# Labbeti/conette-audio-captioning

Measured on AMD Instinct MI355X. Metric: clips_per_sec, higher is better.
Workload: dtype bf16; 1 GPU; B=64/GPU x 10 s @ 32 kHz clips, ConvNeXt encoder + beam-3 KV-cached decode (min 3 / max 20 tokens, V=5631), synthetic seeded checkpoint; batch_per_gpu=64, global_batch=64, beam_size=3, parallelism=dp1, world_size_observed=1, allreduce_of_ones=1, decode_group=2, decode_streams=2, encode_streams=1, input_batches_rotated=4

## Files before the change

conette-audio-captioning_amd/csrc/common.h:

```cpp
#pragma once
#include <hip/hip_runtime.h>
#include <stdint.h>
#include <stdio.h>
#include <string.h>
#include <mutex>
#include <set>
#include <utility>

typedef __bf16 bf16_t;
typedef __attribute__((ext_vector_type(8))) __bf16 bf16x8;
typedef __attribute__((ext_vector_type(4))) __bf16 bf16x4;
typedef __attribute__((ext_vector_type(4))) float f32x4;
typedef __attribute__((ext_vector_type(16))) float f32x16;

typedef _Float16 half_t;
template <typename H> using cn_h8 = H __attribute__((ext_vector_type(8)));
template <typename H> using cn_h4 = H __attribute__((ext_vector_type(4)));
typedef _Float16 cn_h2 __attribute__((ext_vector_type(2)));
template <typename T> struct CnIsH16 { static constexpr bool value = false; };
template <> struct CnIsH16<bf16_t> { static constexpr bool value = true; };
template <> struct CnIsH16<half_t> { static constexpr bool value = true; };
__device__ __forceinline__ f32x16 cn_mma32(cn_h8<bf16_t> a, cn_h8<bf16_t> b, f32x16 c) {
  return __builtin_amdgcn_mfma_f32_32x32x16_bf16(a, b, c, 0, 0, 0);
}
__device__ __forceinline__ f32x16 cn_mma32(cn_h8<half_t> a, cn_h8<half_t> b, f32x16 c) {
  return __builtin_amdgcn_mfma_f32_32x32x16_f16(a, b, c, 0, 0, 0);
}
__device__ __forceinline__ f32x4 cn_mma16(cn_h8<bf16_t> a, cn_h8<bf16_t> b, f32x4 c) {
  return __builtin_amdgcn_mfma_f32_16x16x32_bf16(a, b, c, 0, 0, 0);
}
__device__ __forceinline__ f32x4 cn_mma16(cn_h8<half_t> a, cn_h8<half_t> b, f32x4 c) {
  return __builtin_amdgcn_mfma_f32_16x16x32_f16(a, b, c, 0, 0, 0);
}
template <typename H> __device__ __forceinline__ cn_h8<H> cn_sat8(cn_h8<H> v) {
  if constexpr (__is_same(H, half_t)) {
    cn_h8<H> m;
#pragma unroll
    for (int i = 0; i < 8; ++i) m[i] = (H)65504.0f;
    return __builtin_elementwise_min(v, m);
  }
  return v;
}
template <typename H> __device__ __forceinline__ cn_h8<H> cn_pack8(float a, float b, float c, float d, float e, float f, float g, float h) {
  return cn_h8<H>{(H)a, (H)b, (H)c, (H)d, (H)e, (H)f, (H)g, (H)h};
}

__device__ __forceinline__ unsigned cn_lds_addr(const void* p) {
  return (unsigned)(size_t)(const __attribute__((address_space(3))) char*)p;
}
__device__ __forceinline__ void cn_dma16_v(const void* src_lane, unsigned lds) {
  asm volatile("s_mov_b32 m0, %1\n\tglobal_load_lds_dwordx4 %0, off" ::"v"(src_lane), "s"(lds) : "memory", "m0");
}
__device__ __forceinline__ void cn_dma16_s(const void* src_base, unsigned voff, unsigned lds) {
  asm volatile("s_mov_b32 m0, %2\n\tglobal_load_lds_dwordx4 %0, %1" ::"v"(voff), "s"(src_base), "s"(lds) : "memory", "m0");
}
__device__ __forceinline__ void cn_vm_wait(int n) {
#define CN_VM_CASE(N) case N: asm volatile("s_waitcnt vmcnt(" #N ")" ::: "memory"); break;
  switch (n) {
    CN_VM_CASE(0) CN_VM_CASE(1) CN_VM_CASE(2) CN_VM_CASE(3) CN_VM_CASE(4) CN_VM_CASE(5) CN_VM_CASE(6) CN_VM_CASE(7)
    CN_VM_CASE(8) CN_VM_CASE(9) CN_VM_CASE(10) CN_VM_CASE(11) CN_VM_CASE(12) CN_VM_CASE(13) CN_VM_CASE(14) CN_VM_CASE(15)
    CN_VM_CASE(16) CN_VM_CASE(17) CN_VM_CASE(18) CN_VM_CASE(19) CN_VM_CASE(20) CN_VM_CASE(21) CN_VM_CASE(22) CN_VM_CASE(23)
    CN_VM_CASE(24) CN_VM_CASE(25) CN_VM_CASE(26) CN_VM_CASE(27) CN_VM_CASE(28) CN_VM_CASE(29) CN_VM_CASE(30) CN_VM_CASE(31)
    CN_VM_CASE(32) CN_VM_CASE(33) CN_VM_CASE(34) CN_VM_CASE(35) CN_VM_CASE(36) CN_VM_CASE(37) CN_VM_CASE(38) CN_VM_CASE(39)
    CN_VM_CASE(40) CN_VM_CASE(41) CN_VM_CASE(42) CN_VM_CASE(43) CN_VM_CASE(44) CN_VM_CASE(45) CN_VM_CASE(46) CN_VM_CASE(47)
    CN_VM_CASE(48) CN_VM_CASE(49) CN_VM_CASE(50) CN_VM_CASE(51) CN_VM_CASE(52) CN_VM_CASE(53) CN_VM_CASE(54) CN_VM_CASE(55)
    CN_VM_CASE(56) CN_VM_CASE(57) CN_VM_CASE(58) CN_VM_CASE(59) CN_VM_CASE(60) CN_VM_CASE(61) CN_VM_CASE(62)
    default: break;
  }
#undef CN_VM_CASE
}

typedef __attribute__((ext_vector_type(2))) float f32x2;
typedef __attribute__((ext_vector_type(8))) _Float16 f16x8;
typedef __attribute__((ext_vector_type(4))) unsigned u32x4;

struct sp16_t {
  _Float16 hi, lo;
};
__device__ __forceinline__ unsigned cn_sp16_bits(float x) {
  x = __builtin_amdgcn_fmed3f(x, -65504.0f, 65504.0f);
  const _Float16 hi = (_Float16)x;
  const _Float16 lo = (_Float16)(x - (float)hi);
  return (unsigned)__builtin_bit_cast(unsigned short, hi) | ((unsigned)__builtin_bit_cast(unsigned short, lo) << 16);
}
__device__ __forceinline__ float cn_sp16_value(unsigned w) {
  return (float)__builtin_bit_cast(_Float16, (unsigned short)(w & 0xffffu)) + (float)__builtin_bit_cast(_Float16, (unsigned short)(w >> 16));
}

#define CN_OK 0
#define CN_ERR_ARG 1
#define CN_ERR_HIP 2
#define CN_ERR_WEIGHT 3
#define CN_ERR_WORKSPACE 4

void cn_set_error(const char* fmt, ...);

#define CN_HIP(expr)                                                                      \
  do {                                                                                    \
    hipError_t _e = (expr);                                                               \
    if (_e != hipSuccess) {                                                               \
      cn_set_error("%s:%d %s -> %s", __FILE__, __LINE__, #expr, hipGetErrorString(_e));   \
      return CN_ERR_HIP;                                                                  \
    }                                                                                     \
  } while (0)

#define CN_LAUNCH_CHECK()                                                                 \
  do {                                                                                    \
    hipError_t _e = hipGetLastError();                                                    \
    if (_e != hipSuccess) {                                                               \
      cn_set_error("%s:%d launch -> %s", __FILE__, __LINE__, hipGetErrorString(_e));      \
      return CN_ERR_HIP;                                                                  \
    }                                                                                     \
  } while (0)

#define CN_TRY(expr)                 \
  do {                               \
    int _s = (expr);                 \
    if (_s != CN_OK) return _s;      \
  } while (0)

static inline int cn_configure_lds(const void* fn, int bytes) {
  static std::mutex mu;
  static std::set<std::pair<int, const void*>> done;
  int dev = 0;
  CN_HIP(hipGetDevice(&dev));
  std::lock_guard<std::mutex> lock(mu);
  if (done.count(std::make_pair(dev, fn))) return CN_OK;
  CN_HIP(hipFuncSetAttribute(fn, hipFuncAttributeMaxDynamicSharedMemorySize, bytes));
  done.insert(std::make_pair(dev, fn));
  return CN_OK;
}

static inline size_t cn_align(size_t x, size_t a = 256) { return (x + a - 1) / a * a; }
static inline int cn_cdiv(int a, int b) { return (a + b - 1) / b; }

template <typename T> __device__ __forceinline__ T cn_from_f32(float x);
template <> __device__ __forceinline__ float cn_from_f32<float>(float x) { return x; }
template <> __device__ __forceinline__ bf16_t cn_from_f32<bf16_t>(float x) { return (bf16_t)x; }
template <> __device__ __forceinline__ half_t cn_from_f32<half_t>(float x) { return (half_t)__builtin_amdgcn_fmed3f(x, -65504.0f, 65504.0f); }
template <> __device__ __forceinline__ sp16_t cn_from_f32<sp16_t>(float x) { return __builtin_bit_cast(sp16_t, cn_sp16_bits(x)); }
__device__ __forceinline__ float cn_to_f32(float x) { return x; }
__device__ __forceinline__ float cn_to_f32(bf16_t x) { return (float)x; }
__device__ __forceinline__ float cn_to_f32(half_t x) { return (float)x; }
__device__ __forceinline__ float cn_to_f32(sp16_t x) { return (float)x.hi + (float)x.lo; }

__device__ __forceinline__ float cn_ld1(const float* p) { return *p; }
__device__ __forceinline__ float cn_ld1(const half_t* p) { return (float)*p; }
__device__ __forceinline__ f32x4 cn_ld4(const float* p) { return *(const f32x4*)p; }
__device__ __forceinline__ f32x4 cn_ld4(const half_t* p) {
  const cn_h4<half_t> h = *(const cn_h4<half_t>*)p;
  return f32x4{(float)h[0], (float)h[1], (float)h[2], (float)h[3]};
}

__device__ __forceinline__ float cn_gelu(float x) { return 0.5f * x * (1.0f + erff(x * 0.70710678118654752440f)); }

__device__ __forceinline__ float cn_gelu_fast(float x) {
  const float z = fabsf(x) * 0.70710678118654752440f;
  const float t = __builtin_amdgcn_rcpf(fmaf(0.3275911f, z, 1.0f));
  float p = fmaf(1.061405429f, t, -1.453152027f);
  p = fmaf(p, t, 1.421413741f);
  p = fmaf(p, t, -0.284496736f);
  p = fmaf(p, t, 0.254829592f);
  const float e = 1.0f - p * t * __expf(-z * z);
  return 0.5f * x + 0.5f * fabsf(x) * e;
}

__device__ __forceinline__ f32x2 cn_gelu_fast2(f32x2 x) {
  const f32x2 ax = __builtin_elementwise_abs(x);
  const f32x2 d = ax * (0.70710678118654752440f * 0.3275911f) + 1.0f;
  const f32x2 t = f32x2{__builtin_amdgcn_rcpf(d[0]), __builtin_amdgcn_rcpf(d[1])};
  f32x2 p = t * 1.061405429f + (-1.453152027f);
  p = p * t + 1.421413741f;
  p = p * t + (-0.284496736f);
  p = p * t + 0.254829592f;
  const f32x2 u = x * 0.84932180028801904272f;
  const f32x2 zz = -(u * u);
  const f32x2 e = f32x2{__builtin_amdgcn_exp2f(zz[0]), __builtin_amdgcn_exp2f(zz[1])};
  const f32x2 er = 1.0f - (p * t) * e;
  const f32x2 h = x * 0.5f;
  return __builtin_elementwise_abs(h) * er + h;
}
__device__ __forceinline__ f32x2 cn_gelu_as2(f32x2 x) {
  const f32x2 ax = __builtin_elementwise_abs(x);
  const f32x2 d = ax * (0.70710678118654752440f * 0.3275911f) + 1.0f;
  const f32x2 t = f32x2{__builtin_amdgcn_rcpf(d[0]), __builtin_amdgcn_rcpf(d[1])};
  f32x2 p = t * 1.061405429f + (-1.453152027f);
  p = p * t + 1.421413741f;
  p = p * t + (-0.284496736f);
  p = p * t + 0.254829592f;
  const f32x2 u = x * 0.84932180028801904272f;
  const f32x2 zz = -(u * u);
  const f32x2 e = f32x2{__builtin_amdgcn_exp2f(zz[0]), __builtin_amdgcn_exp2f(zz[1])};
  const f32x2 q = (p * t) * e;
  const f32x2 pos = f32x2{fmaxf(x[0], 0.f), fmaxf(x[1], 0.f)};
  return pos - (ax * 0.5f) * q;
}
__device__ __forceinline__ float cn_gelu_as(float x) { return cn_gelu_as2(f32x2{x, x})[0]; }
__device__ __forceinline__ f32x4 cn_gelu_as4(f32x4 x) {
  const f32x2 a = cn_gelu_as2(f32x2{x[0], x[1]}), b = cn_gelu_as2(f32x2{x[2], x[3]});
  return f32x4{a[0], a[1], b[0], b[1]};
}
__device__ __forceinline__ f32x4 cn_gelu_fast4(f32x4 x) {
  const f32x2 a = cn_gelu_fast2(f32x2{x[0], x[1]}), b = cn_gelu_fast2(f32x2{x[2], x[3]});
  return f32x4{a[0], a[1], b[0], b[1]};
}

template <int DEG> __device__ __forceinline__ float cn_gelu_e1_half(float h) {
  const float a = __builtin_fabsf(h);
  float p;
  if constexpr (DEG == 3) {
    p = fmaf(a, 8.0f * -0.02487156353890896f, 4.0f * -0.49887558817863464f);
    p = fmaf(p, a, 2.0f * -1.1291841268539429f);
    p = fmaf(p, a, 1.0f - 1.0035500526428223f);
  } else {
    static_assert(DEG == 5, "degree 3 or 5");
    p = fmaf(a, 32.0f * -0.0004728270578198135f, 16.0f * 0.007081141695380211f);
    p = fmaf(p, a, 8.0f * -0.05181875079870224f);
    p = fmaf(p, a, 4.0f * -0.4600019156932831f);
    p = fmaf(p, a, 2.0f * -1.1507835388183594f);
    p = fmaf(p, a, 1.0f - 1.0000382661819458f);
  }
  float g = fmaf(-a, __builtin_amdgcn_exp2f(p), h + a);
  asm("" : "+v"(g));
  return g;
}
// ... 74 lines not shown
```

conette-audio-captioning_amd/csrc/ctx.h:

```cpp
#pragma once
#include "../../include/conette_hip.h"
#include "common.h"

#define CN_N_MELS 224
#define CN_N_FFT 1024
#define CN_HOP 320
#define CN_N_BINS 513
#define CN_N_TAGS 527
#define CN_FEAT 768
#define CN_MAX_LAYERS 12

static const int CN_DEPTHS[4] = {3, 3, 9, 3};
static const int CN_DIMS[4] = {96, 192, 384, 768};

struct CnBlockW {
  const float* dw_w;
  const unsigned* dw_wp;
  const float* dw_b;
  const float* ln_w;
  const float* ln_b;
  const void* w1;
  const float* b1;
  const void* w2;
  const float* b2;
  const float* scale;
  const void* mlp_stream;
  const void* mlp_sp;
};

struct CnDownW {
  const float* ln_w;
  const float* ln_b;
  const void* w;
  const float* bias;
  const void* fused;
};

struct CnLayerW {
  const void* sa_in_w;
  const float* sa_in_b;
  const void* sa_out_w;
  const float* sa_out_b;
  const void* ca_q_w;
  const float* ca_q_b;
  const void* ca_out_w;
  const float* ca_out_b;
  const void* ff1_w;
  const float* ff1_b;
  const void* ff2_w;
  const float* ff2_b;
  const float *n1w, *n1b, *n2w, *n2b, *n3w, *n3b;
  const void* blk_w;
  const void* ffn_w;
  const float* blk_p;
};

struct CnRuntime;

struct conette_ctx {
  conette_config cfg;
  CnRuntime* rt;
  void* dec_graphs;
  unsigned long long serial;
  uint32_t prof_mask;
  int dec_unfused;
  int esize;
  int sp16;
  int f16;
  int no_encoder;
  const float* window;
  const float2* tw512;
  const float2* tw1024;
  const int* band;
  int mel_rows;
  const float* melC;
  const float* bn_scale;
  const float* bn_shift;
  const float* stem_w;
  const float* stem_b;
  const float* stem_ln_w;
  const float* stem_ln_b;
  CnBlockW blocks[18];
  CnDownW down[3];
  const float* norm_w;
  const float* norm_b;
  const void* head_w;
  const float* head_b;
  const void* proj_w;
  const float* proj_b;
  const void* kv_w;
  const float* kv_b;
  CnLayerW layers[CN_MAX_LAYERS];
  const float* emb;
  const float* pe;
  int pe_len;
  const void* cls_w;
  const float* cls_b;
  int n_cu;
  int enc_reserved_cus;
  int forcing_stepwise;
  int score_vsplit;
  char* arena;
  size_t arena_bytes;
  size_t arena_used;
};

void cn_prof_begin(conette_ctx* ctx, int cls, hipStream_t s);
void cn_prof_end(conette_ctx* ctx, int cls, hipStream_t s);
struct CnProfScope {
  conette_ctx* ctx;
  int cls;
  hipStream_t s;
  CnProfScope(conette_ctx* c, int k, hipStream_t st) : ctx(c), cls(k), s(st) {
    if (ctx->prof_mask & (1u << cls)) cn_prof_begin(ctx, cls, s);
  }
  ~CnProfScope() {
    if (ctx->prof_mask & (1u << cls)) cn_prof_end(ctx, cls, s);
  }
};

int cn_frontend(conette_ctx* ctx, const float* wave, int B, int L, float* out, hipStream_t s);

#define CN_BY_PRECISION(ctx, ...)                                                          \
  do {                                                                                     \
    switch ((ctx)->cfg.precision) {                                                        \
      case CONETTE_PREC_BF16: { typedef bf16_t OT; return __VA_ARGS__; }                   \
      case CONETTE_PREC_F16: { typedef half_t OT; return __VA_ARGS__; }                    \
      case CONETTE_PREC_F16X2: { typedef sp16_t OT; return __VA_ARGS__; }                  \
      default: { typedef float OT; return __VA_ARGS__; }                                   \
    }                                                                                      \
  } while (0)
#define CN_H16_CALL(ctx, ...)                          \
  do {                                                 \
    if ((ctx)->f16) { typedef half_t HT; __VA_ARGS__; } \
    else { typedef bf16_t HT; __VA_ARGS__; }            \
  } while (0)
```

conette-audio-captioning_amd/csrc/decoder.hip:

```cpp
#include "ctx.h"
#include <stdlib.h>

#include <type_traits>

#include "gemm2.h"
#include "dec_ffn.h"
#include "dec_score.h"
#include "dec_rows.h"
#include "dec_search.h"
#include "dec_sample.h"
#include "dec_group.h"
#include "dec_constrain.h"
#include "dec_require.h"
#include "dec_align.h"
#include "dec_ensemble.h"

#define FF2_SPLITS 8
static int ff2_splits_default() { return 4; }


struct DecWs {
  void *fe_t, *mem, *kvc, *xt, *attn_t, *ffh, *kc, *vc;
  float *x, *x2, *qkv, *q, *tmp, *logits, *slabs;
  int *n_active, *slot, *prefix, *anc, *cur_tok, *out_len, *eos_idx;
// ... 368 lines not shown
    if (step == 0 && a.step0_logits)
      CN_HIP(hipMemcpyAsync(a.step0_logits, w.logits, (size_t)R * w.ldv * 4, hipMemcpyDeviceToDevice, s));
    if (forcing) {
      hipLaunchKernelGGL(cn_force_store_kernel, dim3(cn_cdiv(V, 1024), R), dim3(256), 0, s, w.logits, w.ldv, V, maxp, step,
                         a.force_logits);
      CN_LAUNCH_CHECK();
      continue;
    }
    if (a.greedy_logits) {
      hipLaunchKernelGGL(cn_greedy_logits_kernel, dim3(cn_cdiv(V, 1024), B), dim3(256), 0, s, ss, step, cfg.pad_id, a.greedy_logits);
      CN_LAUNCH_CHECK();
    }
    CnProfScope ps_search(ctx, CONETTE_PROF_SEARCH, s);
    if (sampling) {
      SmArgs sa;
      sa.logits = w.logits, sa.forbid = a.forbid, sa.uniforms = a.uniforms, sa.prefix = w.prefix, sa.cur_tok = w.cur_tok;
      sa.sum_lp = w.sum_lp, sa.fin = w.slot, sa.live = w.live, sa.preds = a.mult_preds, sa.sum_out = a.mult_lprobs;
      sa.lens = a.sample_lens, sa.sizes = a.out_sizes, sa.tok_lp = a.sample_tok_lp, sa.step_logits = a.sample_step_logits;
      sa.ldv = w.ldv, sa.V = V, sa.R = R, sa.maxp = maxp, sa.min_pred = min_pred, sa.eos_id = cfg.eos_id, sa.top_k = a.top_k;
      sa.temperature = a.temperature, sa.top_p = a.top_p;
      const int vpt = cn_cdiv(V, SM_T);
#define SM_LAUNCH(VPT_) hipLaunchKernelGGL((cn_sample_step_kernel<VPT_>), dim3(R), dim3(SM_T), 0, s, sa, step)
      if (vpt <= 2) SM_LAUNCH(2);
      else if (vpt <= 4) SM_LAUNCH(4);
      else if (vpt <= 6) SM_LAUNCH(6);
      else if (vpt <= SM_VPT) SM_LAUNCH(8);
      else SM_LAUNCH(0);
#undef SM_LAUNCH
      CN_LAUNCH_CHECK();
      continue;
    }
    if (grouped) {
      cn_group_step_launch(ss, gs, B, step, s);
      CN_LAUNCH_CHECK();
      continue;
    }
    if (a.constrained) {
      if (a.req_width > 0) cn_require_step_launch(ss, cs, rq, B, step, s);
      else cn_constrain_step_launch(ss, cs, B, step, s);
      CN_LAUNCH_CHECK();
      continue;
    }
    if (V <= S3_T * S3_VPT && beam <= 8) {
#define S3_LAUNCH(NR_, VPT_) hipLaunchKernelGGL((cn_search_step3_kernel<NR_, VPT_>), dim3(B), dim3(S3_T), 0, s, ss, step)
      const int vpt = cn_cdiv(V, S3_T);
      if (beam <= 4) {
        if (vpt <= 2) S3_LAUNCH(4, 2);
        else if (vpt <= 4) S3_LAUNCH(4, 4);
        else if (vpt <= 6) S3_LAUNCH(4, 6);
        else S3_LAUNCH(4, 8);
      } else {
        if (vpt <= 4) S3_LAUNCH(8, 4);
        else S3_LAUNCH(8, 8);
      }
#undef S3_LAUNCH
    } else {
      hipLaunchKernelGGL(cn_search_step_kernel, dim3(B), dim3(256), 0, s, ss, step);
    }
    CN_LAUNCH_CHECK();
  }
  if (forcing || sampling) return CN_OK;
  hipLaunchKernelGGL(cn_finalize_kernel, dim3(cn_cdiv(B, 64)), dim3(64), 0, s, B, beam, maxp, cfg.eos_id, a.mult_preds,
                     a.mult_lprobs, w.out_len, a.best_preds, a.best_lprobs, w.eos_idx, a.out_sizes, a.margins);
  CN_LAUNCH_CHECK();
  hipLaunchKernelGGL(cn_finalize2_kernel, dim3(1), dim3(256), 0, s, B, w.eos_idx, a.out_sizes);
  CN_LAUNCH_CHECK();
  return CN_OK;
}

struct DecGraph {
  DecArgs key;
  hipGraphExec_t exec;
  hipGraph_t graph;
  hipEvent_t last;
  int seen;
  int nodes;
};
static void dec_graph_release(DecGraph& g) {
  if (!g.exec) return;
  if (g.last) {
    if (hipEventSynchronize(g.last) != hipSuccess) (void)hipGetLastError();
    (void)hipEventDestroy(g.last);
  }
  (void)hipGraphExecDestroy(g.exec);
  (void)hipGraphDestroy(g.graph);
  g.exec = nullptr, g.graph = nullptr, g.last = nullptr;
}
#define CN_MAX_DEC_GRAPHS 64
struct DecGraphCache {
  std::mutex mu;
  DecGraph g[CN_MAX_DEC_GRAPHS] = {};
  int n = 0;
  int enabled = 1;
  int last_nodes = 0;
};
static std::mutex g_dec_cache_create_mu;
static DecGraphCache* graph_cache(conette_ctx* ctx, bool create) {
  std::lock_guard<std::mutex> lock(g_dec_cache_create_mu);
  if (ctx->dec_graphs == nullptr && create) ctx->dec_graphs = new DecGraphCache();
  return (DecGraphCache*)ctx->dec_graphs;
}
void cn_decode_graphs_free(conette_ctx* ctx) {
  DecGraphCache* c = graph_cache(ctx, false);
  if (!c) return;
  {
    std::lock_guard<std::mutex> lock(c->mu);
    for (int i = 0; i < c->n; ++i) dec_graph_release(c->g[i]);
    c->n = 0;
  }
  std::lock_guard<std::mutex> lock(g_dec_cache_create_mu);
  delete c;
  ctx->dec_graphs = nullptr;
}
extern "C" int conette_set_option(conette_ctx* ctx, int32_t option, int32_t value) {
  if (!ctx) return CN_ERR_ARG;
  if (option == CONETTE_OPT_DECODE_GRAPH) {
    DecGraphCache* c = graph_cache(ctx, true);
    if (c) {
      std::lock_guard<std::mutex> lock(c->mu);
      c->enabled = value ? 1 : 0;
    }
    return CN_OK;
  }
  if (option == CONETTE_OPT_DECODE_FUSION) {
    ctx->dec_unfused = value ? 0 : 1;
    DecGraphCache* c = graph_cache(ctx, false);
    if (c) {
      std::lock_guard<std::mutex> lock(c->mu);
      for (int i = 0; i < c->n; ++i) dec_graph_release(c->g[i]);
      c->n = 0;
    }
    return CN_OK;
  }
  if (option == CONETTE_OPT_FORCING_STEPWISE) {
    ctx->forcing_stepwise = value ? 1 : 0;
    return CN_OK;
  }
  if (option == CONETTE_OPT_SCORE_VSPLIT) {
    if (value < 0) {
      cn_set_error("set_option: score vocabulary split %d < 0", value);
      return CN_ERR_ARG;
    }
    ctx->score_vsplit = value;
    return CN_OK;
  }
  if (option == CONETTE_OPT_ENCODE_RESERVED_CUS) {
    if (value < 0 || value > ctx->n_cu / 2) {
      cn_set_error("set_option: reserved CUs %d outside 0 .. %d", value, ctx->n_cu / 2);
      return CN_ERR_ARG;
    }
    ctx->enc_reserved_cus = value;
    return CN_OK;
  }
  cn_set_error("set_option: unknown option %d", option);
  return CN_ERR_ARG;
}

template <typename... A>
static int dec_check_model(const conette_ctx* ctx, const char* who, int len, int min_pred, const char* len_fmt, A... len_args) {
  if (len < 1 || len > CN_MAX_PRED || len > ctx->pe_len || min_pred < 0) {
    cn_set_error(len_fmt, len_args...);
    return CN_ERR_ARG;
  }
  if (ctx->cfg.d_model != 256 || ctx->cfg.nhead != 8) {
    cn_set_error("%s: kernels are specialised for d_model=256, nhead=8", who);
    return CN_ERR_ARG;
  }
  return CN_OK;
}
static int dec_check_workspace(const char* who, size_t workspace_bytes, size_t need) {
  if (workspace_bytes < need) {
    cn_set_error("%s: workspace %zu < %zu", who, workspace_bytes, need);
    return CN_ERR_WORKSPACE;
  }
  return CN_OK;
}

static int dec_check_search(const char* who, const int32_t* frame_lens, int batch, int t_audio, int beam, int min_pred, int max_pred,
                            const int32_t* best_preds, const float* best_lprobs, const int32_t* mult_preds, const float* mult_lprobs,
                            const int32_t* out_sizes) {
  if (!frame_lens || !best_preds || !best_lprobs || !mult_preds || !mult_lprobs || !out_sizes || batch <= 0 || t_audio <= 0) {
    cn_set_error("%s: bad argument", who);
    return CN_ERR_ARG;
  }
  if (beam < 1 || beam > CN_MAX_BEAM || max_pred < 1 || max_pred > CN_MAX_PRED || min_pred < 0) {
    cn_set_error("%s: beam=%d (1..%d) max_pred=%d (1..%d) min_pred=%d unsupported", who, beam, CN_MAX_BEAM, max_pred, CN_MAX_PRED,
                 min_pred);
    return CN_ERR_ARG;
  }
  return CN_OK;
}
static int dec_check_member(const char* who, const conette_ctx* ctx, int min_pred, int max_pred, size_t workspace_bytes, size_t need) {
  CN_TRY(dec_check_model(ctx, who, max_pred, min_pred, "%s: max_pred exceeds positional table", who));
  return dec_check_workspace(who, workspace_bytes, need);
}

template <typename Run>
static int dec_graph_run(conette_ctx* ctx, const DecArgs& key, hipStream_t s, Run run) {
  DecGraphCache* cache = graph_cache(ctx, true);
  const uint32_t dec_classes = (1u << CONETTE_PROF_DEC_PREPARE) | (1u << CONETTE_PROF_DEC_GEMM) |
                               (1u << CONETTE_PROF_DEC_ATTN) | (1u << CONETTE_PROF_DEC_MISC) |
                               (1u << CONETTE_PROF_SEARCH);
  if (!cache || (ctx->prof_mask & dec_classes) != 0) return run();

  auto find = [&]() -> DecGraph* {
    for (int i = 0; i < cache->n; ++i)
      if (cache->g[i].key == key) {
        const DecGraph hit = cache->g[i];
        memmove(&cache->g[i], &cache->g[i + 1], sizeof(DecGraph) * (cache->n - 1 - i));
        cache->g[cache->n - 1] = hit;
        return &cache->g[cache->n - 1];
      }
    return nullptr;
  };
  enum { EAGER, CAPTURE } todo = EAGER;
  DecGraph evicted;
  memset(&evicted, 0, sizeof(evicted));
  {
    std::lock_guard<std::mutex> lock(cache->mu);
    if (!cache->enabled) {
      todo = EAGER;
    } else if (DecGraph* e = find()) {
      if (e->exec) {
        CN_HIP(hipGraphLaunch(e->exec, s));
        CN_HIP(hipEventRecord(e->last, s));
        cache->last_nodes = e->nodes;
        return CN_OK;
      }
      if (e->seen == 1) {
        e->seen = 2;
        todo = CAPTURE;
      }
    } else {
      if (cache->n == CN_MAX_DEC_GRAPHS) {
        evicted = cache->g[0];
        memmove(&cache->g[0], &cache->g[1], sizeof(DecGraph) * (CN_MAX_DEC_GRAPHS - 1));
        cache->n--;
      }
      DecGraph* fresh = &cache->g[cache->n++];
      memset(fresh, 0, sizeof(*fresh));
      memcpy(&fresh->key, &key, sizeof(key));
      fresh->seen = 1;
    }
  }
  dec_graph_release(evicted);
  if (todo == EAGER) return run();

  hipGraph_t graph = nullptr;
  hipGraphExec_t exec = nullptr;
  hipEvent_t last = nullptr;
  auto capture = [&]() -> bool {
    if (hipStreamBeginCapture(s, hipStreamCaptureModeRelaxed) != hipSuccess) return false;
    const int rc = run();
    if (hipStreamEndCapture(s, &graph) != hipSuccess || rc != CN_OK || graph == nullptr) return false;
    if (hipGraphInstantiate(&exec, graph, nullptr, nullptr, 0) != hipSuccess || exec == nullptr) return false;
    return hipEventCreateWithFlags(&last, hipEventDisableTiming) == hipSuccess;
  };
  if (!capture()) {
    (void)hipGetLastError();
    if (exec) (void)hipGraphExecDestroy(exec);
    if (graph) (void)hipGraphDestroy(graph);
    {
      std::lock_guard<std::mutex> lock(cache->mu);
      cache->enabled = 0;
    }
    return run();
  }
  size_t n_nodes = 0;
  if (hipGraphGetNodes(graph, nullptr, &n_nodes) != hipSuccess) (void)hipGetLastError();
  {
    std::lock_guard<std::mutex> lock(cache->mu);
    DecGraph* e = find();
    if (e && !e->exec) {
      e->exec = exec, e->graph = graph, e->last = last, e->nodes = (int)n_nodes;
      cache->last_nodes = e->nodes;
      CN_HIP(hipGraphLaunch(exec, s));
      CN_HIP(hipEventRecord(last, s));
      return CN_OK;
    }
  }
  CN_HIP(hipGraphLaunch(exec, s));
  CN_HIP(hipEventRecord(last, s));
  DecGraph tmp;
  memset(&tmp, 0, sizeof(tmp));
  tmp.exec = exec, tmp.graph = graph, tmp.last = last;
  dec_graph_release(tmp);
  return CN_OK;
}

extern "C" int conette_decode(conette_ctx* ctx, const float* frame_embs, const int32_t* frame_lens,
                              const int32_t* bos_ids, const uint8_t* forbid_mask, int32_t batch, int32_t t_audio,
                              int32_t beam, int32_t min_pred, int32_t max_pred, int32_t* best_preds,
                              float* best_lprobs, int32_t* mult_preds, float* mult_lprobs, int32_t* out_sizes,
                              float* step0_logits, int32_t* trace_sel, float* trace_val, float* margins,
                              void* workspace, size_t workspace_bytes, void* stream) {
  if (!ctx || !frame_embs || !bos_ids || !workspace) {
    cn_set_error("decode: bad argument");
    return CN_ERR_ARG;
  }
  CN_TRY(dec_check_search("decode", frame_lens, batch, t_audio, beam, min_pred, max_pred, best_preds, best_lprobs, mult_preds, mult_lprobs,
                          out_sizes));
  CN_TRY(dec_check_member("decode", ctx, min_pred, max_pred, workspace_bytes, conette_decode_workspace_bytes(ctx, batch, t_audio, beam, max_pred)));
  DecArgs a;
  memset(&a, 0, sizeof(a));
  a.frame_embs = frame_embs, a.frame_lens = frame_lens, a.bos_ids = bos_ids, a.forbid = forbid_mask;
  a.best_preds = best_preds, a.best_lprobs = best_lprobs, a.mult_preds = mult_preds, a.mult_lprobs = mult_lprobs;
// ... 573 lines not shown
```

conette-audio-captioning_amd/csrc/encoder.hip:

```cpp
#include <stddef.h>

#include "ctx.h"
#include <type_traits>

__device__ int g_cn_nonfinite;
__device__ __forceinline__ void cn_watch_stat(float v) {
  if (!(__builtin_fabsf(v) <= 3.0e38f)) atomicAdd(&g_cn_nonfinite, 1);
}

#include "gemm2.h"
#include "mlp_rc2.h"
#include "mlp_rs16.h"
#include "mlp_sp.h"
#include "down_fused.h"

template <typename XT>
__global__ __launch_bounds__(256) void cn_stem_mfma_kernel(const float* __restrict__ in, int F, int H0, long n_pos,
                                                           const float* __restrict__ w , const float* __restrict__ bias,
                                                           const float* __restrict__ ln_w, const float* __restrict__ ln_b,
                                                           XT* __restrict__ out) {
  __shared__ __attribute__((aligned(16))) float s_p[3 * 96];
  for (int i = threadIdx.x; i < 3 * 96; i += 256) s_p[i] = i < 96 ? bias[i] : i < 192 ? ln_w[i - 96] : ln_b[i - 192];
  const int lane = threadIdx.x & 63, j = lane & 31, h = lane >> 5;
  float a[3][8];
#pragma unroll
  for (int t = 0; t < 3; ++t)
#pragma unroll
    for (int s = 0; s < 8; ++s) a[t][s] = w[(4 * (s >> 1) + 2 * h + (s & 1)) * 96 + 32 * t + cn_rc2_chan(j)];
  __syncthreads();
  const long n_tiles = (n_pos + 31) >> 5;
  const long n_waves = (long)gridDim.x * 4;
  for (long tile = (long)blockIdx.x * 4 + (threadIdx.x >> 6); tile < n_tiles; tile += n_waves) {
    const long pos = tile * 32 + j;
    const long p = pos < n_pos ? pos : n_pos - 1;
    const int wq = (int)(p % 56);
    const long tt = p / 56;
    const int hh = (int)(tt % H0);
    const int b = (int)(tt / H0);
    f32x2 xv[4];
#pragma unroll
    for (int i = 0; i < 4; ++i) {
      const int r = 4 * hh - 4 + i;
      xv[i] = f32x2{0.f, 0.f};
      if (r >= 0 && r < F) xv[i] = *(const f32x2*)(in + ((size_t)b * F + r) * CN_N_MELS + 4 * wq + 2 * h);
    }
    f32x16 acc[3];
#pragma unroll
    for (int t = 0; t < 3; ++t)
#pragma unroll
      for (int u = 0; u < 2; ++u) {
        const f32x4 b0 = *(const f32x4*)(s_p + 32 * t + 16 * u + 8 * h), b1 = *(const f32x4*)(s_p + 32 * t + 16 * u + 8 * h + 4);
#pragma unroll
        for (int e = 0; e < 4; ++e) acc[t][8 * u + e] = b0[e], acc[t][8 * u + 4 + e] = b1[e];
      }
#pragma unroll
    for (int s = 0; s < 8; ++s)
#pragma unroll
      for (int t = 0; t < 3; ++t) acc[t] = __builtin_amdgcn_mfma_f32_32x32x2f32(a[t][s], xv[s >> 1][s & 1], acc[t], 0, 0, 0);
    float sum = 0.f;
#pragma unroll
    for (int t = 0; t < 3; ++t)
#pragma unroll
      for (int r = 0; r < 16; ++r) sum += acc[t][r];
    sum += __shfl_xor(sum, 32);
    const float mean = sum * (1.0f / 96.0f);
    float v2 = 0.f;
#pragma unroll
    for (int t = 0; t < 3; ++t)
#pragma unroll
      for (int r = 0; r < 16; ++r) {
        acc[t][r] -= mean;
        v2 = fmaf(acc[t][r], acc[t][r], v2);
      }
    v2 += __shfl_xor(v2, 32);
    const float rstd = 1.0f / sqrtf(v2 * (1.0f / 96.0f) + 1e-6f);
    if (pos < n_pos) {
      XT* o = out + (size_t)pos * 96 + 8 * h;
#pragma unroll
      for (int t = 0; t < 3; ++t)
#pragma unroll
        for (int u = 0; u < 2; ++u) {
          const int ch = 32 * t + 16 * u + 8 * h;
          float v[8];
#pragma unroll
          for (int q = 0; q < 2; ++q) {
            const f32x4 lw = *(const f32x4*)(s_p + 96 + ch + 4 * q), lb = *(const f32x4*)(s_p + 192 + ch + 4 * q);
#pragma unroll
            for (int e = 0; e < 4; ++e) v[4 * q + e] = acc[t][8 * u + 4 * q + e] * rstd * lw[e] + lb[e];
          }
          if constexpr (sizeof(XT) == 2) {
            *(cn_h8<XT>*)(o + 32 * t + 16 * u) = cn_h8<XT>{cn_from_f32<XT>(v[0]), cn_from_f32<XT>(v[1]), cn_from_f32<XT>(v[2]), cn_from_f32<XT>(v[3]),
                                                          cn_from_f32<XT>(v[4]), cn_from_f32<XT>(v[5]), cn_from_f32<XT>(v[6]), cn_from_f32<XT>(v[7])};
          } else {
            *(f32x4*)(o + 32 * t + 16 * u) = f32x4{v[0], v[1], v[2], v[3]};
            *(f32x4*)(o + 32 * t + 16 * u + 4) = f32x4{v[4], v[5], v[6], v[7]};
          }
        }
    }
  }
}

__device__ unsigned long long g_dw_prof[8];
#define DW_STAMP(i)                                                   \
  if (dbg) {                                                          \
    const unsigned long long t_ = clock64();                          \
    if ((threadIdx.x & 63) == 0) atomicAdd(&g_dw_prof[i], t_ - t_prev); \
    t_prev = t_;                                                      \
  }

template <int C, int S, int TH> struct DwTile {
  static constexpr int NCHUNK = C / 4;
  static constexpr int PITCH4 = NCHUNK | 1;
  static constexpr int PITCH = PITCH4 * 4;
};

template <typename T, typename XT, int C, int S, int TH>
__global__ __launch_bounds__((C > 384 ? 384 : C) * S) void cn_dwconv_ln_kernel(const XT* __restrict__ x, int H, int W, int tiles_h,
                                                            int tiles_w, const float* __restrict__ dw_w ,
                                                            const unsigned* __restrict__ dw_wp ,
                                                            const float* __restrict__ dw_b,
                                                            const float* __restrict__ ln_w,
                                                            const float* __restrict__ ln_b, T* __restrict__ y,
                                                            int dbg) {
  extern __shared__ __attribute__((aligned(16))) char smem_raw[];
  float* s_v = (float*)smem_raw;
  unsigned long long t_prev = dbg ? clock64() : 0;
  constexpr int NP = TH * 4;
  constexpr int CT = C > 384 ? 384 : C;
  constexpr int PITCH = DwTile<C, S, TH>::PITCH;
  const int tid = threadIdx.x;
  const int c0 = tid % CT, sidx = tid / CT;
  int bid = cn_xcd_remap(blockIdx.x, gridDim.x);
  const int tw = bid % tiles_w;
  bid /= tiles_w;
  const int th = bid % tiles_h;
  const int b = bid / tiles_h;
  const int h0 = th * TH, w0 = tw * (4 * S) + sidx * 4;

  int wcl[10];
  bool wok[10];
#pragma unroll
  for (int q = 0; q < 10; ++q) {
    const int ww = w0 - 3 + q;
    wok[q] = (ww >= 0) && (ww < W);
    wcl[q] = min(max(ww, 0), W - 1) * C;
  }
#pragma unroll 1
  for (int c = c0; c < C; c += CT) {
  float acc[TH][4];
  const float bias = dw_b[c];
#pragma unroll
  for (int a = 0; a < TH; ++a)
#pragma unroll
    for (int e = 0; e < 4; ++e) acc[a][e] = bias;
  const XT* xb = x + (size_t)b * H * W * C + c;
  const bool interior = (h0 >= 3) && (h0 + TH + 3 <= H) && (w0 >= 3) && (w0 + 4 + 3 <= W);
  if constexpr (sizeof(XT) == 2) {
    static_assert(TH % 2 == 0, "row pairs");
    cn_h2 ke[3][7], ko[3][7];
#pragma unroll
    for (int a = 0; a < 3; ++a)
#pragma unroll
      for (int j = 0; j < 7; ++j) {
        ke[a][j] = __builtin_bit_cast(cn_h2, dw_wp[(a * 7 + j) * C + c]);
        ko[a][j] = __builtin_bit_cast(cn_h2, dw_wp[(21 + a * 7 + j) * C + c]);
      }
    DW_STAMP(0)
    auto fma_pair = [&](int r, const cn_h2 (&p)[10]) {
#pragma unroll
      for (int oh = 0; oh < TH; ++oh) {
        const int i = r - oh;
        if (i < -1 || i > 6) continue;
#pragma unroll
        for (int q = 0; q < 10; ++q)
#pragma unroll
          for (int ow = 0; ow < 4; ++ow) {
            const int j = q - ow;
            if (j < 0 || j > 6) continue;
            if (i == -1) acc[oh][ow] = fmaf((float)p[q][1], (float)ke[0][j][0], acc[oh][ow]);
            else if (i == 6) acc[oh][ow] = fmaf((float)p[q][0], (float)ko[2][j][1], acc[oh][ow]);
            else if ((i & 1) == 0) acc[oh][ow] = __builtin_amdgcn_fdot2(p[q], ke[i >> 1][j], acc[oh][ow], false);
            else acc[oh][ow] = __builtin_amdgcn_fdot2(p[q], ko[i >> 1][j], acc[oh][ow], false);
          }
      }
    };
    constexpr int NPR = (TH + 6) / 2;
    if (interior) {
      const XT* base = xb + ((size_t)(h0 - 3) * W + (w0 - 3)) * C;
      auto load_pair = [&](int r, cn_h2 (&p)[10]) {
        const XT* x0 = base + (size_t)r * W * C;
        const XT* x1 = x0 + (size_t)W * C;
#pragma unroll
        for (int q = 0; q < 10; ++q) p[q] = cn_h2{x0[q * C], x1[q * C]};
      };
      cn_h2 pa[10], pb[10];
      load_pair(0, pa);
#pragma unroll
      for (int u = 0; u < NPR; u += 2) {
        if (u + 1 < NPR) load_pair(2 * (u + 1), pb);
        fma_pair(2 * u, pa);
        if (u + 2 < NPR) load_pair(2 * (u + 2), pa);
        if (u + 1 < NPR) fma_pair(2 * (u + 1), pb);
      }
    } else {
#pragma unroll
      for (int u = 0; u < NPR; ++u) {
        const int hh0 = h0 - 3 + 2 * u, hh1 = hh0 + 1;
        const bool ok0 = (hh0 >= 0) && (hh0 < H), ok1 = (hh1 >= 0) && (hh1 < H);
        const XT* x0 = xb + (size_t)min(max(hh0, 0), H - 1) * W * C;
        const XT* x1 = xb + (size_t)min(max(hh1, 0), H - 1) * W * C;
        XT v0[10], v1[10];
#pragma unroll
        for (int q = 0; q < 10; ++q) v0[q] = x0[wcl[q]], v1[q] = x1[wcl[q]];
        cn_h2 p[10];
#pragma unroll
        for (int q = 0; q < 10; ++q) p[q] = cn_h2{(ok0 && wok[q]) ? v0[q] : (XT)0.f, (ok1 && wok[q]) ? v1[q] : (XT)0.f};
        fma_pair(2 * u, p);
      }
    }
  } else {
  float k[49];
#pragma unroll
  for (int i = 0; i < 49; ++i) k[i] = dw_w[i * C + c];
  DW_STAMP(0)
  auto fma_row = [&](int r, const XT (&v)[10]) {
#pragma unroll
    for (int oh = 0; oh < TH; ++oh) {
      const int i = r - oh;
      if (i < 0 || i > 6) continue;
#pragma unroll
      for (int q = 0; q < 10; ++q)
#pragma unroll
        for (int ow = 0; ow < 4; ++ow) {
          const int j = q - ow;
          if (j < 0 || j > 6) continue;
          acc[oh][ow] = fmaf((float)v[q], k[i * 7 + j], acc[oh][ow]);
        }
    }
  };
  if (interior) {
    const XT* base = xb + ((size_t)(h0 - 3) * W + (w0 - 3)) * C;
    XT va[10], vb[10];
#pragma unroll
    for (int q = 0; q < 10; ++q) va[q] = base[q * C];
#pragma unroll
    for (int r = 0; r < TH + 6; r += 2) {
      if (r + 1 < TH + 6) {
        const XT* xr = base + (size_t)(r + 1) * W * C;
#pragma unroll
        for (int q = 0; q < 10; ++q) vb[q] = xr[q * C];
      }
// ... 444 lines not shown
  }
  if (__syncthreads_or(bad ? 1 : 0) && threadIdx.x == 0) atomicAdd(&g_cn_nonfinite, 1);
}

template <typename T>
__global__ __launch_bounds__(256) void cn_clip_pool_ln_kernel(const float* __restrict__ fe, int Tn,
                                                              const float* __restrict__ ln_w,
                                                              const float* __restrict__ ln_b, T* __restrict__ out) {
  __shared__ float s_red[8];
  const int b = blockIdx.x, tid = threadIdx.x;
  float v[3];
  float s = 0.f;
#pragma unroll
  for (int i = 0; i < 3; ++i) {
    const int c = tid + 256 * i;
    float mx = -INFINITY, sm = 0.f;
    const float* col = fe + (size_t)b * Tn * CN_FEAT + c;
    int t = 0;
    for (; t + 8 <= Tn; t += 8) {
      float a[8];
#pragma unroll
      for (int u = 0; u < 8; ++u) a[u] = col[(size_t)(t + u) * CN_FEAT];
#pragma unroll
      for (int u = 0; u < 8; ++u) {
        mx = fmaxf(mx, a[u]);
        sm += a[u];
      }
    }
    for (; t < Tn; ++t) {
      const float a = col[(size_t)t * CN_FEAT];
      mx = fmaxf(mx, a);
      sm += a;
    }
    v[i] = mx + sm / (float)Tn;
    s += v[i];
  }
  s = cn_wave_sum(s);
  if ((tid & 63) == 0) s_red[tid >> 6] = s;
  __syncthreads();
  const float mean = (s_red[0] + s_red[1] + s_red[2] + s_red[3]) * (1.0f / CN_FEAT);
  float s2 = 0.f;
#pragma unroll
  for (int i = 0; i < 3; ++i) {
    const float d = v[i] - mean;
    s2 = fmaf(d, d, s2);
  }
  s2 = cn_wave_sum(s2);
  if ((tid & 63) == 0) s_red[4 + (tid >> 6)] = s2;
  __syncthreads();
  const float rstd = 1.0f / sqrtf((s_red[4] + s_red[5] + s_red[6] + s_red[7]) * (1.0f / CN_FEAT) + 1e-6f);
#pragma unroll
  for (int i = 0; i < 3; ++i) {
    const int c = tid + 256 * i;
    out[(size_t)b * CN_FEAT + c] = cn_from_f32<T>((v[i] - mean) * rstd * ln_w[c] + ln_b[c]);
  }
}

#ifndef CN_SP_NW96
#define CN_SP_NW96 12
#define CN_SP_NST96 4
#endif

struct EncGeom {
  int F, H[4], W[4];
};
static EncGeom enc_geom(int L) {
  EncGeom g;
  g.F = L / CN_HOP + 1;
  g.H[0] = (g.F + 8 - 4) / 4 + 1;
  g.W[0] = 56;
  for (int i = 1; i < 4; ++i) {
    g.H[i] = g.H[i - 1] / 2;
    g.W[i] = g.W[i - 1] / 2;
  }
  return g;
}

extern "C" int32_t conette_num_frames(int32_t n_samples) { return n_samples / CN_HOP + 1; }
extern "C" int32_t conette_num_audio_frames(int32_t n_samples) { return enc_geom(n_samples).H[3]; }

struct EncWs {
  float* logmel;
  void* x;
  void* y;
  void* h;
  void* fe_t;
  void* clip_t;
  size_t total;
};
static EncWs enc_ws(const conette_ctx* ctx, int B, int L, char* base) {
  const EncGeom g = enc_geom(L);
  const size_t es = ctx->esize;
  const size_t n0 = (size_t)B * g.H[0] * g.W[0] * 96;
  EncWs w;
  size_t off = 0;
  auto take = [&](size_t bytes) {
    char* p = base ? base + off : nullptr;
    off += cn_align(bytes);
    return p;
  };
  w.logmel = (float*)take((size_t)B * g.F * CN_N_MELS * 4);
  w.x = take((n0 + 32 * 96) * 4);
  w.y = take((n0 + 32 * 96) * es);
  w.h = take(n0 * 4 * es);
  w.fe_t = take((size_t)B * g.H[3] * CN_FEAT * es);
  w.clip_t = take((size_t)B * CN_FEAT * es);
  w.total = off;
  return w;
}

extern "C" size_t conette_encode_workspace_bytes(const conette_ctx* ctx, int32_t batch, int32_t n_samples) {
  return enc_ws(ctx, batch, n_samples, nullptr).total;
}

template <typename T, typename XT>
static int dwconv_dispatch(int C, const XT* x, int B, int H, int W, const CnBlockW& bw, T* y, hipStream_t s) {
  switch (C) {
    case 96: return launch_dwconv<T, XT, 96, CN_DW96_S, sizeof(XT) == 2 ? CN_DW96_TH : 8>(x, B, H, W, bw, y, s);
    case 192: return launch_dwconv<T, XT, 192, CN_DW192_S, sizeof(XT) == 2 ? CN_DW192_TH : 8>(x, B, H, W, bw, y, s);
    case 384:
      if (W == 14) return launch_dwconv_fw<T, XT, 384, 14, CN_FW_TH, CN_FW_SPLIT>(x, B, H, bw, y, s);
      return launch_dwconv<T, XT, 384, 1, 4>(x, B, H, W, bw, y, s);
    case 768:
      if (W == 7) return launch_dwconv_fw<T, XT, 768, 7, 4>(x, B, H, bw, y, s);
      return launch_dwconv<T, XT, 768, 1, 4>(x, B, H, W, bw, y, s);
  }
  cn_set_error("dwconv: unsupported C=%d", C);
  return CN_ERR_ARG;
}

static int tap_copy(float* dst, const float* src, size_t n, hipStream_t s) {
  if (dst) CN_HIP(hipMemcpyAsync(dst, src, n * sizeof(float), hipMemcpyDeviceToDevice, s));
  return CN_OK;
}
static __global__ void cn_tap_widen_kernel(const half_t* __restrict__ src, float* __restrict__ dst, size_t n) {
  for (size_t i = (size_t)blockIdx.x * blockDim.x + threadIdx.x; i < n; i += (size_t)gridDim.x * blockDim.x) dst[i] = (float)src[i];
}
static int tap_copy(float* dst, const half_t* src, size_t n, hipStream_t s) {
  if (dst) {
    hipLaunchKernelGGL(cn_tap_widen_kernel, dim3((unsigned)((n + 255) / 256 < 4096 ? (n + 255) / 256 : 4096)), dim3(256), 0, s, src, dst, n);
    CN_LAUNCH_CHECK();
  }
  return CN_OK;
}

template <typename T, typename XT>
static int encode_impl(conette_ctx* ctx, const float* wave, int B, int L, float* frame_embs, float* clip_probs,
                       const conette_encode_taps* taps, char* wsp, hipStream_t s) {
  const EncGeom g = enc_geom(L);
  EncWs ws = enc_ws(ctx, B, L, wsp);
  T* y = (T*)ws.y;
  T* hbuf = (T*)ws.h;
  XT* const wsx = (XT*)ws.x;
  {
    CnProfScope ps(ctx, CONETTE_PROF_FRONTEND, s);
    CN_TRY(cn_frontend(ctx, wave, B, L, ws.logmel, s));
  }
  if (taps) CN_TRY(tap_copy(taps->logmel, ws.logmel, (size_t)B * g.F * CN_N_MELS, s));
  {
    const long n_pos = (long)B * g.H[0] * g.W[0];
    CnProfScope ps(ctx, CONETTE_PROF_STEM, s);
    const long n_tiles = (n_pos + 31) / 32;
    const unsigned grid = (unsigned)std::min<long>((n_tiles + 3) / 4, 8L * ctx->n_cu);
    hipLaunchKernelGGL((cn_stem_mfma_kernel<XT>), dim3(grid), dim3(256), 0, s, ws.logmel, g.F, g.H[0], n_pos, ctx->stem_w, ctx->stem_b,
                       ctx->stem_ln_w, ctx->stem_ln_b, wsx);
    CN_LAUNCH_CHECK();
    if (taps) CN_TRY(tap_copy(taps->stem, wsx, (size_t)n_pos * 96, s));
  }
  XT* xc = wsx;
  int blk = 0;
  for (int st = 0; st < 4; ++st) {
    const int C = CN_DIMS[st], H = g.H[st], W = g.W[st];
    const long P = (long)B * H * W;
    if (st > 0) {
      const int Cp = CN_DIMS[st - 1], Hp = g.H[st - 1], Wp = g.W[st - 1];
      const long n_in = (long)B * Hp * Wp;
      const CnDownW& dw = ctx->down[st - 1];
      CnProfScope ps(ctx, CONETTE_PROF_DOWNSAMPLE, s);
      bool fused_down = false;
      if constexpr (CnIsH16<T>::value) if (Cp <= 192 && dw.fused != nullptr) {
        XT* xo = xc == wsx ? (XT*)ws.h : wsx;
        const int nb = ctx->n_cu - ctx->enc_reserved_cus;
        if (Cp == 96) CN_TRY((cn_launch_down_fused<96, 8, T, XT>(xc, B, Hp, Wp, dw.fused, xo, nb, s)));
        else CN_TRY((cn_launch_down_fused_ring<192, 4, 4, 3, T, XT>(xc, B, Hp, Wp, dw.fused, xo, nb, s)));
        xc = xo;
        if (taps) CN_TRY(tap_copy(taps->down[st], xc, (size_t)P * C, s));
        fused_down = true;
      }
      if (!fused_down) {
      const int ppb = Cp == 96 ? 32 : 16;
      const dim3 pg((unsigned)((n_in + ppb - 1) / ppb));
      if (Cp == 96)
        hipLaunchKernelGGL((cn_ln_patchify_kernel<T, XT, 96>), pg, dim3(256), 0, s, xc, Hp, Wp, n_in, dw.ln_w, dw.ln_b, y);
      else if (Cp == 192)
        hipLaunchKernelGGL((cn_ln_patchify_kernel<T, XT, 192>), pg, dim3(256), 0, s, xc, Hp, Wp, n_in, dw.ln_w, dw.ln_b, y);
      else
        hipLaunchKernelGGL((cn_ln_patchify_kernel<T, XT, 384>), pg, dim3(256), 0, s, xc, Hp, Wp, n_in, dw.ln_w, dw.ln_b, y);
      CN_LAUNCH_CHECK();
      EpiBiasAct<XT, ACT_NONE> epi{dw.bias, wsx, C, ACT_NONE};
      CN_TRY(cn_mm(y, 4 * Cp, (const T*)dw.w, 4 * Cp, (int)P, C, 4 * Cp, epi, s));
      xc = wsx;
      if (taps) CN_TRY(tap_copy(taps->down[st], xc, (size_t)P * C, s));
      }
    }
    for (int b = 0; b < CN_DEPTHS[st]; ++b, ++blk) {
      const CnBlockW& bw = ctx->blocks[blk];
      {
        CnProfScope ps(ctx, CONETTE_PROF_DWCONV_LN, s);
        CN_TRY((dwconv_dispatch<T, XT>(C, xc, B, H, W, bw, y, s)));
      }
      bool fused = false;
      if constexpr (std::is_same<T, sp16_t>::value) {
        if (bw.mlp_sp != nullptr && C <= 192) {
          CnProfScope ps(ctx, CONETTE_PROF_PW1_GEMM, s);
          const int nb = ctx->n_cu - ctx->enc_reserved_cus;
          if (C == 96) CN_TRY((cn_launch_mlp_sp_ring<96, CN_SP_NW96, CN_SP_NST96>(y, bw.mlp_sp, xc, (int)P, nb, s)));
          else CN_TRY((cn_launch_mlp_sp_ring<192, 8, 3>(y, bw.mlp_sp, xc, (int)P, nb, s)));
          fused = true;
        }
      }
      if constexpr (CnIsH16<T>::value) if (!fused) {
        if (bw.mlp_stream != nullptr && C <= 384) {
          CnProfScope ps(ctx, CONETTE_PROF_PW1_GEMM, s);
          const T* wsm = (const T*)bw.mlp_stream;
          if (C == 96) CN_TRY((cn_launch_mlp_rc2_resident<96, 12, 1>(y, wsm, xc, (int)P, ctx->n_cu - ctx->enc_reserved_cus, s)));
          else if (C == 192) CN_TRY((cn_launch_mlp_rc2_ring<192, 8, CN_RC2_NCK(192), CN_RC2_NCK(192) == 2 ? 3 : 5>(y, wsm, xc, (int)P, ctx->n_cu - ctx->enc_reserved_cus, s)));
          else CN_TRY((cn_launch_mlp_rs16<384, 4, 3, 8>(y, wsm, xc, (int)P, ctx->n_cu - ctx->enc_reserved_cus, s)));
          fused = true;
        }
      }
      if (!fused) {
        {
          CnProfScope ps(ctx, CONETTE_PROF_PW1_GEMM, s);
          constexpr int kAct = CnGeluAct<T>::value;
          EpiBiasAct<T, kAct> e1{bw.b1, hbuf, 4 * C, kAct};
          CN_TRY(cn_mm(y, C, (const T*)bw.w1, C, (int)P, 4 * C, C, e1, s));
        }
        {
          CnProfScope ps(ctx, CONETTE_PROF_PW2_GEMM, s);
          EpiResidT<XT> e2{bw.b2, bw.scale, xc, xc, C};
          CN_TRY(cn_mm(hbuf, 4 * C, (const T*)bw.w2, 4 * C, (int)P, C, 4 * C, e2, s));
        }
      }
      if (taps && b == 0) CN_TRY(tap_copy(taps->stage_block0[st], xc, (size_t)P * C, s));
      if (taps && taps->struct_bytes >= offsetof(conette_encode_taps, block) + (size_t)(blk + 1) * sizeof(float*))
        CN_TRY(tap_copy(taps->block[blk], xc, (size_t)P * C, s));
    }
    if (taps) CN_TRY(tap_copy(taps->stage[st], xc, (size_t)P * C, s));
  }
  const int Tn = g.H[3];
  CnProfScope ps_heads(ctx, CONETTE_PROF_HEADS, s);
  hipLaunchKernelGGL((cn_frame_mean_kernel<T, XT>), dim3((unsigned)(B * Tn)), dim3(256), 0, s, xc, g.W[3], CN_FEAT,
                     frame_embs, (T*)nullptr);
  CN_LAUNCH_CHECK();
  if (clip_probs) {
    hipLaunchKernelGGL((cn_clip_pool_ln_kernel<T>), dim3((unsigned)B), dim3(256), 0, s, frame_embs, Tn, ctx->norm_w,
                       ctx->norm_b, (T*)ws.clip_t);
    CN_LAUNCH_CHECK();
    EpiBiasAct<float> eh{ctx->head_b, clip_probs, CN_N_TAGS, ACT_SIGMOID};
    CN_TRY(cn_mm((const T*)ws.clip_t, CN_FEAT, (const T*)ctx->head_w, CN_FEAT, B, CN_N_TAGS, CN_FEAT, eh, s));
  }
  return CN_OK;
}

extern "C" int conette_encode_nonfinite(conette_ctx* ctx, void* stream, int32_t* count) {
  if (!ctx || !count) {
    cn_set_error("encode_nonfinite: bad argument");
    return CN_ERR_ARG;
  }
  hipStream_t s = (hipStream_t)stream;
  int32_t host = 0;
  CN_HIP(hipMemcpyFromSymbolAsync(&host, HIP_SYMBOL(g_cn_nonfinite), sizeof(host), 0, hipMemcpyDeviceToHost, s));
  CN_HIP(hipStreamSynchronize(s));
  if (host != 0) {
    const int32_t zero = 0;
    CN_HIP(hipMemcpyToSymbolAsync(HIP_SYMBOL(g_cn_nonfinite), &zero, sizeof(zero), 0, hipMemcpyHostToDevice, s));
    CN_HIP(hipStreamSynchronize(s));
  }
  *count = host;
  return CN_OK;
}

extern "C" int conette_frontend_logmel(conette_ctx* ctx, const float* wave, int32_t batch, int32_t n_samples,
                                       float* out, void* stream) {
  if (!ctx || !wave || !out || batch <= 0) {
    cn_set_error("frontend_logmel: bad argument");
    return CN_ERR_ARG;
  }
  if (ctx->no_encoder) {
    cn_set_error("frontend_logmel: decoder-only context (created without preprocessor.encoder.* tensors)");
    return CN_ERR_ARG;
  }
  return cn_frontend(ctx, wave, batch, n_samples, out, (hipStream_t)stream);
}

extern "C" int conette_encode(conette_ctx* ctx, const float* wave, int32_t batch, int32_t n_samples,
                              float* frame_embs, float* clip_probs, const conette_encode_taps* taps, void* workspace,
                              size_t workspace_bytes, void* stream) {
  if (conette_num_audio_frames(n_samples) < 1) {
    cn_set_error("encode: n_samples=%d is too short: the encoder's three 2x downsamplings need >= 7680 samples "
                 "(0.24 s at 32 kHz) to leave one audio frame", n_samples);
    return CN_ERR_ARG;
  }
  if (!ctx || !wave || !frame_embs || !workspace || batch <= 0) {
    cn_set_error("encode: bad argument");
    return CN_ERR_ARG;
  }
  if (ctx->no_encoder) {
    cn_set_error("encode: decoder-only context (created without preprocessor.encoder.* tensors: a BaselinePLM-layout checkpoint "
                 "takes precomputed frame embeddings)");
    return CN_ERR_ARG;
  }
  if (taps && taps->struct_bytes < offsetof(conette_encode_taps, block)) {
    cn_set_error("encode: conette_encode_taps.struct_bytes = %zu is smaller than the version-1 members (%zu): set it to "
                 "sizeof(conette_encode_taps)", taps->struct_bytes, offsetof(conette_encode_taps, block));
    return CN_ERR_ARG;
  }
  const size_t need = conette_encode_workspace_bytes(ctx, batch, n_samples);
  if (workspace_bytes < need) {
    cn_set_error("encode: workspace %zu < %zu", workspace_bytes, need);
    return CN_ERR_WORKSPACE;
// ... 13 lines not shown
```

conette-audio-captioning_amd/csrc/frontend.hip:

```cpp
#include "ctx.h"

__device__ __forceinline__ float2 cmul(float2 a, float2 b) { return float2{a.x * b.x - a.y * b.y, a.x * b.y + a.y * b.x}; }
__device__ __forceinline__ float2 cadd(float2 a, float2 b) { return float2{a.x + b.x, a.y + b.y}; }
__device__ __forceinline__ float2 csub(float2 a, float2 b) { return float2{a.x - b.x, a.y - b.y}; }
__device__ __forceinline__ float2 cmul_mi(float2 a) { return float2{a.y, -a.x}; }

__device__ __forceinline__ void dft8(float2 (&v)[8]) {
  const float h = 0.70710678118654752440f;
  float2 a[8];
#pragma unroll
  for (int i = 0; i < 4; ++i) {
    a[i] = cadd(v[i], v[i + 4]);
    a[i + 4] = csub(v[i], v[i + 4]);
  }
  a[5] = float2{h * (a[5].x + a[5].y), h * (a[5].y - a[5].x)};
  a[6] = cmul_mi(a[6]);
  a[7] = float2{h * (a[7].y - a[7].x), -h * (a[7].x + a[7].y)};
  float2 b0 = cadd(a[0], a[2]), b2 = csub(a[0], a[2]), b1 = cadd(a[1], a[3]), b3 = cmul_mi(csub(a[1], a[3]));
  float2 b4 = cadd(a[4], a[6]), b6 = csub(a[4], a[6]), b5 = cadd(a[5], a[7]), b7 = cmul_mi(csub(a[5], a[7]));
  v[0] = cadd(b0, b1);
  v[4] = csub(b0, b1);
  v[2] = cadd(b2, b3);
  v[6] = csub(b2, b3);
  v[1] = cadd(b4, b5);
  v[5] = csub(b4, b5);
  v[3] = cadd(b6, b7);
  v[7] = csub(b6, b7);
}

__device__ __forceinline__ void cn_wave_sync() { __builtin_amdgcn_wave_barrier(); }

#define FE_PITCH 72

#ifndef FE_NW
#define FE_NW 16
#endif
#define FE_STATIC_BYTES ((512 + 513) * 8 + 1024 * 4 + FE_NW * 8 * FE_PITCH * 8 + FE_NW * 520 * 4)
#define FE_LDS_TOTAL (160 * 1024)
#define FE_FILL_BYTES ((FE_LDS_TOTAL - FE_STATIC_BYTES - 256) / 256 * 256)
#define FE_MEL_LDS_MAX FE_FILL_BYTES
static_assert(FE_STATIC_BYTES + FE_FILL_BYTES > FE_LDS_TOTAL - 768 && FE_STATIC_BYTES + FE_FILL_BYTES <= FE_LDS_TOTAL,
              "the log-mel block must own its compute unit's LDS");
template <bool MEL_LDS>
__global__ __launch_bounds__(FE_NW * 64) void cn_logmel_kernel(const float* __restrict__ wave, int L, int F, int total, int mel_rows,
                                                        const float* __restrict__ window,
                                                        const float2* __restrict__ tw512,
                                                        const float2* __restrict__ tw1024,
                                                        const float* __restrict__ melC, const int* __restrict__ band,
                                                        const float* __restrict__ bn_scale,
                                                        const float* __restrict__ bn_shift, float* __restrict__ out) {
  __shared__ float2 s_tw512[512];
  __shared__ float2 s_tw1024[513];
  __shared__ __attribute__((aligned(16))) float s_win[1024];
  __shared__ float2 s_x[FE_NW][8 * FE_PITCH];
  __shared__ float s_p[FE_NW][520];
  extern __shared__ __attribute__((aligned(16))) float s_mel[];
  const int tid = threadIdx.x, lane = tid & 63, wv = tid >> 6;
  if (MEL_LDS)
    for (int i = tid; i < mel_rows * CN_N_MELS; i += FE_NW * 64) s_mel[i] = melC[i];
  for (int i = tid; i < 512; i += FE_NW * 64) s_tw512[i] = tw512[i];
  for (int i = tid; i < 513; i += FE_NW * 64) s_tw1024[i] = tw1024[i];
  for (int i = tid; i < 1024; i += FE_NW * 64) s_win[i] = window[i];
  __syncthreads();
  float2* sx = s_x[wv];
  float* sp = s_p[wv];
  int m_lo[4], m_trip[4];
  float m_sc[4], m_sh[4];
#pragma unroll
  for (int g = 0; g < 4; ++g) {
    const int m = lane + 64 * g;
    const bool on = m < CN_N_MELS;
    m_sc[g] = on ? bn_scale[m] : 0.f;
    m_sh[g] = on ? bn_shift[m] : 0.f;
    m_lo[g] = on ? band[2 * m] : 0;
    int nb = on ? band[2 * m + 1] - m_lo[g] : 0;
#pragma unroll
    for (int d = 32; d > 0; d >>= 1) nb = max(nb, __shfl_xor(nb, d));
    m_trip[g] = min(nb, mel_rows);
  }
  const bool pair_loads = (L & 1) == 0 && (((size_t)wave) & 7) == 0;

  for (int base = blockIdx.x * FE_NW; base < total; base += gridDim.x * FE_NW) {
    const int fr = base + wv;
    const bool act = fr < total;
    float2 v[8];
    if (act) {
      const int b = fr / F, f = fr - b * F;
      const float* x = wave + (size_t)b * L;
      const int p0 = f * CN_HOP - CN_N_FFT / 2;
      if (pair_loads && p0 >= 0 && p0 + CN_N_FFT <= L) {
#pragma unroll
        for (int a = 0; a < 8; ++a) {
          const int n2 = 2 * (64 * a + lane);
          const float2 xv = *(const float2*)(x + p0 + n2);
          const float2 wv2 = *(const float2*)(s_win + n2);
          v[a] = float2{xv.x * wv2.x, xv.y * wv2.y};
        }
      } else {
#pragma unroll
        for (int a = 0; a < 8; ++a) {
          const int n2 = 2 * (64 * a + lane);
          int q0 = p0 + n2, q1 = q0 + 1;
          q0 = q0 < 0 ? -q0 : (q0 >= L ? 2 * L - 2 - q0 : q0);
          q1 = q1 < 0 ? -q1 : (q1 >= L ? 2 * L - 2 - q1 : q1);
          v[a] = float2{x[q0] * s_win[n2], x[q1] * s_win[n2 + 1]};
        }
      }
    } else {
#pragma unroll
      for (int a = 0; a < 8; ++a) v[a] = float2{0.f, 0.f};
    }
    dft8(v);
#pragma unroll
    for (int c = 1; c < 8; ++c) v[c] = cmul(v[c], s_tw512[lane * c]);
#pragma unroll
    for (int c = 0; c < 8; ++c) sx[c * FE_PITCH + lane] = v[c];
    cn_wave_sync();
    const int c = lane >> 3, lo3 = lane & 7;
#pragma unroll
    for (int a = 0; a < 8; ++a) v[a] = sx[c * FE_PITCH + 8 * a + lo3];
    dft8(v);
#pragma unroll
    for (int cp = 1; cp < 8; ++cp) v[cp] = cmul(v[cp], s_tw512[8 * lo3 * cp]);
    cn_wave_sync();
#pragma unroll
    for (int cp = 0; cp < 8; ++cp) sx[c * FE_PITCH + cp * 8 + lo3] = v[cp];
    cn_wave_sync();
#pragma unroll
    for (int bp = 0; bp < 8; ++bp) v[bp] = sx[c * FE_PITCH + lo3 * 8 + bp];
    dft8(v);
    cn_wave_sync();
#pragma unroll
    for (int dp = 0; dp < 8; ++dp) sx[c + 8 * lo3 + 64 * dp] = v[dp];
    cn_wave_sync();
#pragma unroll
    for (int j = 0; j < 8; ++j) {
      const int k = lane + 64 * j;
      const float2 A = sx[k];
      const float2 Bz = sx[(512 - k) & 511];
      const float2 E = float2{0.5f * (A.x + Bz.x), 0.5f * (A.y - Bz.y)};
      const float2 O = float2{0.5f * (A.y + Bz.y), -0.5f * (A.x - Bz.x)};
      const float2 X = cadd(E, cmul(s_tw1024[k], O));
      sp[k] = X.x * X.x + X.y * X.y;
    }
    if (lane == 0) {
      const float2 A = sx[0];
      const float xr = A.x - A.y;
      sp[512] = xr * xr;
    }
    cn_wave_sync();
    if (act) {
#pragma unroll
      for (int g = 0; g < 4; ++g) {
        const int m = lane + 64 * g;
        if (m < CN_N_MELS) {
          const int lo = m_lo[g], trip = m_trip[g];
          const float* mc = MEL_LDS ? s_mel : melC;
          float acc = 0.f;
          int i = 0;
          for (; i + 4 <= trip; i += 4) {
            float p[4], w[4];
#pragma unroll
            for (int u = 0; u < 4; ++u) {
              p[u] = sp[min(lo + i + u, CN_N_BINS - 1)];
              w[u] = mc[(i + u) * CN_N_MELS + m];
            }
#pragma unroll
            for (int u = 0; u < 4; ++u) acc = fmaf(p[u], w[u], acc);
          }
          for (; i < trip; ++i) acc = fmaf(sp[min(lo + i, CN_N_BINS - 1)], mc[i * CN_N_MELS + m], acc);
          const float db = 10.0f * log10f(acc < 1e-10f ? 1e-10f : acc);
          out[(size_t)fr * CN_N_MELS + m] = db * m_sc[g] + m_sh[g];
        }
      }
    }
    cn_wave_sync();
  }
}

int cn_frontend(conette_ctx* ctx, const float* wave, int B, int L, float* out, hipStream_t s) {
  if (L <= CN_N_FFT / 2) {
    cn_set_error("frontend: n_samples=%d must exceed %d (reflect padding)", L, CN_N_FFT / 2);
    return CN_ERR_ARG;
  }
  const int F = L / CN_HOP + 1;
  const long total = (long)B * F;
  int grid = (int)((total + FE_NW - 1) / FE_NW);
  if (grid > ctx->n_cu) grid = ctx->n_cu;
  const int mel_bytes = ctx->mel_rows * CN_N_MELS * 4;
  if (mel_bytes <= FE_MEL_LDS_MAX) {
    const int dyn = FE_FILL_BYTES;
    CN_TRY(cn_configure_lds((const void*)cn_logmel_kernel<true>, dyn));
    hipLaunchKernelGGL(cn_logmel_kernel<true>, dim3(grid), dim3(FE_NW * 64), dyn, s, wave, L, F, (int)total, ctx->mel_rows,
                       ctx->window, ctx->tw512, ctx->tw1024, ctx->melC, ctx->band, ctx->bn_scale, ctx->bn_shift, out);
  } else {
    CN_TRY(cn_configure_lds((const void*)cn_logmel_kernel<false>, FE_FILL_BYTES));
    hipLaunchKernelGGL(cn_logmel_kernel<false>, dim3(grid), dim3(FE_NW * 64), FE_FILL_BYTES, s, wave, L, F, (int)total,
                       ctx->mel_rows, ctx->window, ctx->tw512, ctx->tw1024, ctx->melC, ctx->band, ctx->bn_scale, ctx->bn_shift, out);
  }
  CN_LAUNCH_CHECK();
  return CN_OK;
}
```

conette-audio-captioning_amd/csrc/mlp_rc2.h:

```cpp
#pragma once
#include "common.h"

template <int C, int NCK> struct Rc2Geom {
  static constexpr int KS1 = C / 16, NT2 = C / 32, NCH = C / 8;
  static constexpr int F1 = KS1 + 1, F2 = 2 * NT2;
  static constexpr int NSTEP = NCH / NCK;
  static constexpr int FRAGS = NCK * (F1 + F2);
  static constexpr int STEP_BYTES = FRAGS * 1024;
  static constexpr size_t STREAM_BYTES = (size_t)NSTEP * STEP_BYTES;
  static constexpr size_t TOTAL_BYTES = STREAM_BYTES + NT2 * 1024;
};
__host__ __device__ constexpr int cn_rc2_chan(int m) { return (m & 19) | ((m & 4) << 1) | ((m & 8) >> 1); }

#define CN_MLP_XSCALE 0.5f
template <typename HT> __device__ __forceinline__ float cn_gelu_mlp(float x) {
  return cn_gelu_e1_half<__is_same(HT, half_t) ? 5 : 3>(x);
}

template <typename HT>
static __global__ void pk_mlp_rc2(const float* __restrict__ W1, const float* __restrict__ b1, const float* __restrict__ W2,
                           const float* __restrict__ b2, const float* __restrict__ scale, int C, int NCK,
                           HT* __restrict__ dst) {
  const int KS1 = C / 16, NT2 = C / 32, NCH = C / 8, F1 = KS1 + 1, F2 = 2 * NT2, FRAGS = NCK * (F1 + F2), NSTEP = NCH / NCK;
  const int u = blockIdx.x * blockDim.x + threadIdx.x;
  if (u >= (NSTEP * FRAGS + NT2) * 64) return;
  const int l = u & 63, q = (u >> 6) % FRAGS, st = (u >> 6) / FRAGS;
  const int r = l & 31, h = l >> 5;
  float v[8];
  if (st >= NSTEP) {
    const int c = 32 * q + cn_rc2_chan(r);
    const float b = scale[c] * b2[c];
    const float hi = (float)(HT)b;
#pragma unroll
    for (int i = 0; i < 8; ++i) v[i] = 0.f;
    if (h == 0) {
      v[0] = hi;
      v[1] = b - hi;
    }
  } else if (q < NCK * F1) {
    const int j = st * NCK + q / F1, s = q % F1;
    if (s < KS1) {
#pragma unroll
      for (int i = 0; i < 8; ++i) v[i] = CN_MLP_XSCALE * W1[(size_t)(32 * j + r) * C + 16 * s + 8 * h + i];
    } else {
      const float b = CN_MLP_XSCALE * b1[32 * j + r];
      const float hi = (float)(HT)b;
#pragma unroll
      for (int i = 0; i < 8; ++i) v[i] = 0.f;
      if (h == 0) {
        v[0] = hi;
        v[1] = b - hi;
      }
    }
  } else {
    const int q2 = q - NCK * F1;
    const int j = st * NCK + q2 / F2, s = (q2 % F2) / NT2, t = (q2 % F2) % NT2;
    const int c = 32 * t + cn_rc2_chan(r);
    const float sc = scale[c];
#pragma unroll
    for (int i = 0; i < 8; ++i) v[i] = sc * W2[(size_t)c * (4 * C) + 32 * j + 16 * s + 8 * (i >> 2) + 4 * h + (i & 3)];
  }
#pragma unroll
  for (int i = 0; i < 8; ++i) dst[(size_t)u * 8 + i] = (HT)v[i];
}

#define CN_RC2_NCK(C) ((C) == 192 ? 2 : 1)


template <int C, int NCK, typename HT = bf16_t, typename XT = float> struct Rc2Wave {
  typedef Rc2Geom<C, NCK> G;
  typedef cn_h8<HT> hx8;
  static constexpr int KS1 = G::KS1, NT2 = G::NT2, F1 = G::F1, F2 = G::F2;

  static __device__ __forceinline__ hx8 frag(const char* wc, int f) { return *(const hx8*)(wc + f * 1024); }
  static __device__ __forceinline__ f32x16 mma(hx8 a, hx8 b, f32x16 c) { return cn_mma32(a, b, c); }
  static __device__ __forceinline__ hx8 gelu8(const f32x16& X, int o) {
    float g[8];
#pragma unroll
    for (int i = 0; i < 8; ++i) g[i] = cn_gelu_mlp<HT>(X[o + i]);
    return cn_sat8<HT>(cn_pack8<HT>(g[0], g[1], g[2], g[3], g[4], g[5], g[6], g[7]));
  }
  static __device__ __forceinline__ f32x16 zero16() {
    f32x16 z;
#pragma unroll
    for (int i = 0; i < 16; ++i) z[i] = 0.f;
    return z;
  }

  static constexpr int PRE = 4;
  static constexpr int NM = NCK * (F1 + F2), R = PRE + 1;
  struct State {
    hx8 F[R];
    f32x16 X[NCK];
    float g[NCK][16];
    hx8 H[NCK][2];
  };
  static constexpr int gelu_at(int i, int e) {
    if (NCK == 2) return i == 0 ? F1 + 1 + e * (F1 - 1) / 16 : 2 * F1 + e * F2 / 16;
    return e < 8 ? F1 - 1 : F1 + (e - 8) * NT2 / 8;
  }
  template <int Q, int I, int E>
  static __device__ __forceinline__ void gelu_slices(State& st) {
    if constexpr (gelu_at(I, E) == Q) {
      st.g[I][E] = cn_gelu_mlp<HT>(st.X[I][E]);
      if constexpr ((E & 7) == 7) {
        constexpr int o = E - 7;
        st.H[I][E >> 3] = cn_sat8<HT>(cn_pack8<HT>(st.g[I][o], st.g[I][o + 1], st.g[I][o + 2], st.g[I][o + 3],
                                                   st.g[I][o + 4], st.g[I][o + 5], st.g[I][o + 6], st.g[I][o + 7]));
      }
    }
    if constexpr (E + 1 < 16) gelu_slices<Q, I, E + 1>(st);
    else if constexpr (I + 1 < NCK) gelu_slices<Q, I + 1, 0>(st);
  }
  template <int Q>
  static __device__ __forceinline__ void mstep(const char* wc, const hx8 (&fy)[KS1], const hx8 ones, f32x16 (&O)[NT2],
                                               State& st) {
    if constexpr (Q + PRE < NM) st.F[(Q + PRE) % R] = frag(wc, Q + PRE);
    if constexpr (Q < NCK * F1) {
      constexpr int i = Q / F1, s = Q % F1;
      if constexpr (s == 0) st.X[i] = zero16();
      if constexpr (s < KS1) st.X[i] = mma(st.F[Q % R], fy[s], st.X[i]);
      else st.X[i] = mma(st.F[Q % R], ones, st.X[i]);
    } else {
      constexpr int q2 = Q - NCK * F1, i = q2 / F2, k = (q2 % F2) / NT2, t = q2 % NT2;
      O[t] = mma(st.F[Q % R], st.H[i][k], O[t]);
    }
    gelu_slices<Q, 0, 0>(st);
    __builtin_amdgcn_sched_barrier(0);
    if constexpr (Q + 1 < NM) mstep<Q + 1>(wc, fy, ones, O, st);
  }
  template <int Q>
  static __device__ __forceinline__ void prefetch(const char* wc, State& st) {
    st.F[Q % R] = frag(wc, Q);
    if constexpr (Q + 1 < PRE) prefetch<Q + 1>(wc, st);
  }
  static __device__ __forceinline__ void step(const char* wc, const hx8 (&fy)[KS1], const hx8 ones, f32x16 (&O)[NT2]) {
    State st;
    prefetch<0>(wc, st);
    __builtin_amdgcn_sched_barrier(0);
    mstep<0>(wc, fy, ones, O, st);
  }


  static __device__ __forceinline__ void load_y(const HT* __restrict__ Y, int m0, int lane, hx8 (&fy)[KS1]) {
    const HT* base = Y + (size_t)m0 * C;
    const int voff = (lane & 31) * C + 8 * (lane >> 5);
#pragma unroll
    for (int s = 0; s < KS1; ++s) fy[s] = *(const hx8*)(base + voff + 16 * s);
  }

  static __device__ __forceinline__ void init_o(const XT* __restrict__ X, const char* __restrict__ bbf, const hx8 ones, int m0,
                                                int lane, f32x16 (&O)[NT2]) {
    const XT* base = X + (size_t)m0 * C;
    const int voff = (lane & 31) * C + 8 * (lane >> 5);
    hx8 fb[NT2];
    if constexpr (sizeof(XT) == 2) {
      cn_h8<XT> v[NT2][2];
#pragma unroll
      for (int t = 0; t < NT2; ++t) {
        v[t][0] = *(const cn_h8<XT>*)(base + voff + 32 * t);
        v[t][1] = *(const cn_h8<XT>*)(base + voff + 32 * t + 16);
      }
#pragma unroll
      for (int t = 0; t < NT2; ++t) fb[t] = *(const hx8*)(bbf + t * 1024);
#pragma unroll
// ... 224 lines not shown
```

conette-audio-captioning_amd/engine.py:

```python
from __future__ import annotations

import ctypes as C
import os
from typing import Any, Dict, Optional, Tuple

import torch

_HERE = os.path.dirname(os.path.abspath(__file__))
LIB_PATH = os.path.join(_HERE, "libconette_hip.so")

PREC_F32 = 0
PREC_BF16 = 1
PREC_F16X2 = 2
PREC_F16 = 4
N_MELS = 224
FEAT = 768
N_TAGS = 527

EXPORTS = (
    "conette_last_error", "conette_abi_version", "conette_create", "conette_destroy", "conette_num_frames",
    "conette_num_audio_frames", "conette_encode_workspace_bytes", "conette_decode_workspace_bytes",
    "conette_frontend_logmel", "conette_encode", "conette_decode", "conette_resample", "conette_resample_len",
    "conette_set_option", "conette_profile_enable", "conette_profile_read", "conette_stream_create_masked",
    "conette_stream_destroy", "conette_forcing_workspace_bytes", "conette_forcing",
    "conette_greedy_workspace_bytes", "conette_greedy", "conette_decode_graph_nodes", "conette_encode_nonfinite",
    "conette_score_workspace_bytes", "conette_score", "conette_sample_workspace_bytes", "conette_sample",
    "conette_align_workspace_bytes", "conette_align", "conette_decode_groups_workspace_bytes", "conette_decode_groups",
    "conette_decode_constrained_workspace_bytes", "conette_decode_constrained",
    "conette_decode_required_workspace_bytes", "conette_decode_required",
    "conette_decode_ensemble_workspace_bytes", "conette_decode_ensemble",
)
CERT_TOL = {
    "mixed16": {"greedy": (0.032, 0.0, 0.0), "beam": (0.045, 0.0, 0.005), "wide": (0.08, 0.0, 0.005)},
    "f16": {"greedy": (0.063, 0.0, 0.0), "beam": (0.082, 0.0, 0.008), "wide": (0.13, 0.0, 0.008)},
    "bf16+f16dec": {"greedy": (0.20, 0.0, 0.0), "beam": (0.37, 0.0, 0.026), "wide": (0.65, 0.0, 0.05)},
    "bf16": {"greedy": (0.39, 0.0, 0.0), "beam": (0.58, 0.0, 0.05), "wide": (1.0, 0.0, 0.08)},
}


def cert_kind(beam: int) -> str:
    return "greedy" if int(beam) == 1 else ("beam" if int(beam) <= 5 else "wide")


CERT_DEFAULT_BASE = "mixed16"
OPT_DECODE_GRAPH = 1
OPT_DECODE_FUSION = 2
OPT_ENCODE_RESERVED_CUS = 3
OPT_FORCING_STEPWISE = 4
OPT_SCORE_VSPLIT = 5
MAX_DECODE_GRAPHS = 64
PROF_CLASSES = ("frontend", "stem", "dwconv_ln", "pw1_gemm", "pw2_gemm", "downsample", "heads", "dec_prepare",
                "dec_gemm", "dec_attn", "dec_misc", "search")


class ConetteConfigC(C.Structure):
    _fields_ = [(n, C.c_int32) for n in ("precision", "vocab_size", "d_model", "nhead", "n_layers", "d_ff", "pad_id",
                                         "bos_id", "eos_id")] + [("reserved", C.c_int32 * 7)]


class EncodeTapsC(C.Structure):
    _fields_ = [("struct_bytes", C.c_size_t), ("logmel", C.c_void_p), ("stem", C.c_void_p), ("stage_block0", C.c_void_p * 4),
                ("stage", C.c_void_p * 4), ("down", C.c_void_p * 4), ("block", C.c_void_p * 18)]


class ConetteMemberC(C.Structure):
    _fields_ = [("ctx", C.c_void_p), ("frame_embs", C.c_void_p), ("bos_ids", C.c_void_p), ("weight", C.c_float),
                ("workspace", C.c_void_p), ("workspace_bytes", C.c_size_t)]


_lib = None


def load_library() -> C.CDLL:
    global _lib
    if _lib is not None:
        return _lib
    if not os.path.exists(LIB_PATH):
        raise RuntimeError(
            f"{LIB_PATH} is missing: build it with `python -c 'import __graft_entry__ as g; g.build()'` "
            "(the MI355X path has no CPU fallback)")
    lib = C.CDLL(LIB_PATH)
    lib.conette_last_error.restype = C.c_char_p
    lib.conette_abi_version.restype = C.c_int
    lib.conette_create.restype = C.c_int
    lib.conette_create.argtypes = [C.POINTER(ConetteConfigC), C.c_int32, C.POINTER(C.c_char_p), C.POINTER(C.c_void_p),
                                   C.POINTER(C.c_int64), C.POINTER(C.c_void_p)]
    lib.conette_destroy.restype = None
    lib.conette_destroy.argtypes = [C.c_void_p]
    lib.conette_num_frames.restype = C.c_int32
    lib.conette_num_frames.argtypes = [C.c_int32]
    lib.conette_num_audio_frames.restype = C.c_int32
    lib.conette_num_audio_frames.argtypes = [C.c_int32]
    lib.conette_encode_workspace_bytes.restype = C.c_size_t
    lib.conette_encode_workspace_bytes.argtypes = [C.c_void_p, C.c_int32, C.c_int32]
    lib.conette_decode_workspace_bytes.restype = C.c_size_t
    lib.conette_decode_workspace_bytes.argtypes = [C.c_void_p, C.c_int32, C.c_int32, C.c_int32, C.c_int32]
    lib.conette_frontend_logmel.restype = C.c_int
    lib.conette_frontend_logmel.argtypes = [C.c_void_p, C.c_void_p, C.c_int32, C.c_int32, C.c_void_p, C.c_void_p]
    lib.conette_encode.restype = C.c_int
    lib.conette_encode.argtypes = [C.c_void_p, C.c_void_p, C.c_int32, C.c_int32, C.c_void_p, C.c_void_p,
                                   C.POINTER(EncodeTapsC), C.c_void_p, C.c_size_t, C.c_void_p]
    lib.conette_decode.restype = C.c_int
    lib.conette_decode.argtypes = [C.c_void_p, C.c_void_p, C.c_void_p, C.c_void_p, C.c_void_p, C.c_int32, C.c_int32,
                                   C.c_int32, C.c_int32, C.c_int32, C.c_void_p, C.c_void_p, C.c_void_p, C.c_void_p,
                                   C.c_void_p, C.c_void_p, C.c_void_p, C.c_void_p, C.c_void_p, C.c_void_p, C.c_size_t,
                                   C.c_void_p]
    lib.conette_encode_nonfinite.restype = C.c_int
    lib.conette_encode_nonfinite.argtypes = [C.c_void_p, C.c_void_p, C.POINTER(C.c_int32)]
    lib.conette_forcing_workspace_bytes.restype = C.c_size_t
    lib.conette_forcing_workspace_bytes.argtypes = [C.c_void_p, C.c_int32, C.c_int32, C.c_int32]
    lib.conette_forcing.restype = C.c_int
    lib.conette_forcing.argtypes = [C.c_void_p, C.c_void_p, C.c_void_p, C.c_void_p, C.c_int32, C.c_int32, C.c_int32,
                                    C.c_void_p, C.c_void_p, C.c_size_t, C.c_void_p]
    lib.conette_score_workspace_bytes.restype = C.c_size_t
    lib.conette_score_workspace_bytes.argtypes = [C.c_void_p, C.c_int32, C.c_int32, C.c_int32, C.c_int32]
    lib.conette_score.restype = C.c_int
    lib.conette_score.argtypes = [C.c_void_p, C.c_void_p, C.c_void_p, C.c_void_p, C.c_void_p, C.c_int32, C.c_int32, C.c_int32,
                                  C.c_int32, C.c_void_p, C.c_void_p, C.c_void_p, C.c_void_p, C.c_size_t, C.c_void_p]
    lib.conette_align_workspace_bytes.restype = C.c_size_t
    lib.conette_align_workspace_bytes.argtypes = [C.c_void_p, C.c_int32, C.c_int32, C.c_int32, C.c_int32, C.c_int32]
    lib.conette_align.restype = C.c_int
    lib.conette_align.argtypes = [C.c_void_p, C.c_void_p, C.c_void_p, C.c_void_p, C.c_void_p, C.c_int32, C.c_int32, C.c_int32,
                                  C.c_int32, C.c_uint32, C.c_void_p, C.c_void_p, C.c_void_p, C.c_void_p, C.c_void_p, C.c_void_p,
                                  C.c_size_t, C.c_void_p]
    lib.conette_sample_workspace_bytes.restype = C.c_size_t
    lib.conette_sample_workspace_bytes.argtypes = [C.c_void_p, C.c_int32, C.c_int32, C.c_int32, C.c_int32]
    lib.conette_sample.restype = C.c_int
    lib.conette_sample.argtypes = [C.c_void_p, C.c_void_p, C.c_void_p, C.c_void_p, C.c_void_p, C.c_void_p, C.c_int32, C.c_int32,
                                   C.c_int32, C.c_int32, C.c_int32, C.c_float, C.c_int32, C.c_float, C.c_void_p, C.c_void_p,
                                   C.c_void_p, C.c_void_p, C.c_void_p, C.c_void_p, C.c_void_p, C.c_size_t, C.c_void_p]
    lib.conette_decode_groups_workspace_bytes.restype = C.c_size_t
    lib.conette_decode_groups_workspace_bytes.argtypes = [C.c_void_p, C.c_int32, C.c_int32, C.c_int32, C.c_int32, C.c_int32]
    lib.conette_decode_groups.restype = C.c_int
    lib.conette_decode_groups.argtypes = [C.c_void_p, C.c_void_p, C.c_void_p, C.c_void_p, C.c_void_p, C.c_int32, C.c_int32, C.c_int32,
                                          C.c_int32, C.c_float, C.c_int32, C.c_int32, C.c_void_p, C.c_void_p, C.c_void_p, C.c_void_p,
                                          C.c_void_p, C.c_void_p, C.c_void_p, C.c_void_p, C.c_void_p, C.c_size_t, C.c_void_p]
    lib.conette_decode_constrained_workspace_bytes.restype = C.c_size_t
    lib.conette_decode_constrained_workspace_bytes.argtypes = [C.c_void_p, C.c_int32, C.c_int32, C.c_int32, C.c_int32]
    lib.conette_decode_constrained.restype = C.c_int
    lib.conette_decode_constrained.argtypes = [C.c_void_p, C.c_void_p, C.c_void_p, C.c_void_p, C.c_void_p, C.c_void_p, C.c_void_p,
                                               C.c_int32, C.c_void_p, C.c_int32, C.c_int32, C.c_int32, C.c_int32, C.c_int32,
                                               C.c_int32, C.c_void_p, C.c_void_p, C.c_void_p, C.c_void_p, C.c_void_p, C.c_void_p,
                                               C.c_void_p, C.c_void_p, C.c_void_p, C.c_size_t, C.c_void_p]
    lib.conette_decode_required_workspace_bytes.restype = C.c_size_t
    lib.conette_decode_required_workspace_bytes.argtypes = [C.c_void_p, C.c_int32, C.c_int32, C.c_int32, C.c_int32]
    lib.conette_decode_required.restype = C.c_int
    lib.conette_decode_required.argtypes = [C.c_void_p, C.c_void_p, C.c_void_p, C.c_void_p, C.c_void_p, C.c_void_p, C.c_void_p,
                                            C.c_int32, C.c_void_p, C.c_int32, C.c_void_p, C.c_void_p, C.c_int32, C.c_int32, C.c_int32,
                                            C.c_int32, C.c_int32, C.c_int32, C.c_void_p, C.c_void_p, C.c_void_p, C.c_void_p, C.c_void_p,
                                            C.c_void_p, C.c_void_p, C.c_void_p, C.c_void_p, C.c_size_t, C.c_void_p]
    lib.conette_decode_ensemble_workspace_bytes.restype = C.c_size_t
    lib.conette_decode_ensemble_workspace_bytes.argtypes = [C.c_void_p, C.c_int32, C.c_int32, C.c_int32, C.c_int32]
    lib.conette_decode_ensemble.restype = C.c_int
    lib.conette_decode_ensemble.argtypes = [C.POINTER(ConetteMemberC), C.c_int32, C.c_int32, C.c_void_p, C.c_void_p, C.c_int32, C.c_int32,
                                            C.c_int32, C.c_int32, C.c_int32, C.c_void_p, C.c_void_p, C.c_void_p, C.c_void_p, C.c_void_p,
                                            C.c_void_p, C.c_void_p, C.c_void_p, C.c_void_p, C.c_void_p]
    lib.conette_greedy_workspace_bytes.restype = C.c_size_t
    lib.conette_greedy_workspace_bytes.argtypes = [C.c_void_p, C.c_int32, C.c_int32, C.c_int32]
    lib.conette_greedy.restype = C.c_int
    lib.conette_greedy.argtypes = [C.c_void_p, C.c_void_p, C.c_void_p, C.c_void_p, C.c_void_p, C.c_int32, C.c_int32,
                                   C.c_int32, C.c_int32, C.c_void_p, C.c_void_p, C.c_void_p, C.c_void_p, C.c_size_t,
                                   C.c_void_p]
    lib.conette_set_option.restype = C.c_int
    lib.conette_set_option.argtypes = [C.c_void_p, C.c_int32, C.c_int32]
    lib.conette_decode_graph_nodes.restype = C.c_int32
    lib.conette_decode_graph_nodes.argtypes = [C.c_void_p]
    lib.conette_profile_enable.restype = C.c_int
    lib.conette_profile_enable.argtypes = [C.c_void_p, C.c_uint32]
    lib.conette_profile_read.restype = C.c_int
    lib.conette_profile_read.argtypes = [C.c_void_p, C.POINTER(C.c_float), C.POINTER(C.c_int32)]
    lib.conette_stream_create_masked.restype = C.c_int
    lib.conette_stream_create_masked.argtypes = [C.POINTER(C.c_uint32), C.c_int32, C.POINTER(C.c_void_p)]
    lib.conette_stream_destroy.restype = C.c_int
    lib.conette_stream_destroy.argtypes = [C.c_void_p]
    lib.conette_resample.restype = C.c_int
    lib.conette_resample.argtypes = [C.c_void_p, C.c_int32, C.c_int32, C.c_int32, C.c_int32, C.c_void_p, C.c_void_p]
    lib.conette_resample_len.restype = C.c_int32
    lib.conette_resample_len.argtypes = [C.c_int32, C.c_int32, C.c_int32]
    if lib.conette_abi_version() != 3:
        raise RuntimeError("libconette_hip.so ABI version mismatch")
    _lib = lib
    return lib


def _check(status: int, what: str) -> None:
    if status != 0:
        raise RuntimeError(f"{what} failed ({status}): {load_library().conette_last_error().decode()}")


def _stream() -> C.c_void_p:
    return C.c_void_p(torch.cuda.current_stream().cuda_stream)


def _ptr(t: Optional[torch.Tensor]) -> C.c_void_p:
    return C.c_void_p(0 if t is None else t.data_ptr())


def encoder_geometry(n_samples: int) -> Tuple[int, list, list]:
    f = n_samples // 320 + 1
    h = [(f + 8 - 4) // 4 + 1]
    w = [56]
    for _ in range(3):
# ... 5 lines not shown
def make_partitioned_streams(device: torch.device, decode_share: int = 8, n_cus: int = 256):
    lib = load_library()
    words = (n_cus + 31) // 32
    dec = [0] * words
    for i in range(0, n_cus, decode_share):
        dec[i // 32] |= 1 << (i % 32)
    enc = [(~w) & 0xFFFFFFFF for w in dec]
    out = []
    with torch.cuda.device(device):
        for mask in (enc, dec):
            h = C.c_void_p()
            _check(lib.conette_stream_create_masked((C.c_uint32 * words)(*mask), words, C.byref(h)),
                   "conette_stream_create_masked")
            out.append(torch.cuda.ExternalStream(h.value, device=device))
    return out[0], out[1]


def make_masked_stream(device: torch.device, n_share: int, n_cus: int = 256, offset: int = 0):
    lib = load_library()
    words = (n_cus + 31) // 32
    mask = [0] * words
    for j in range(n_share):
        i = (offset + j) % n_cus
        mask[i // 32] |= 1 << (i % 32)
    with torch.cuda.device(device):
        h = C.c_void_p()
        _check(lib.conette_stream_create_masked((C.c_uint32 * words)(*mask), words, C.byref(h)), "conette_stream_create_masked")
        return torch.cuda.ExternalStream(h.value, device=device)


def uncertified_mask(margins: torch.Tensor, best_lprobs: torch.Tensor, tol: Tuple[float, float, float], order: bool = True) -> torch.Tensor:
    a, b, c = tol
    max_pred = margins.shape[2] - 1
    need = a + b * torch.arange(1, max_pred + 1, device=margins.device, dtype=torch.float32)
    ok = (margins[:, 0, :max_pred] >= need).all(dim=1) & (margins[:, 0, max_pred] >= c) & torch.isfinite(best_lprobs)
    if order:
        ok = ok & (margins[:, 1, :max_pred] >= need).all(dim=1)
    return ~ok


def caption_sizes(best_preds: torch.Tensor, mult_preds: torch.Tensor, eos_id: int) -> torch.Tensor:
    max_pred = mult_preds.shape[-1]
    pos = torch.arange(max_pred, device=mult_preds.device)

    def first_eos(x):
        return torch.where(x == eos_id, pos, max_pred).amin(dim=-1)

    ps = torch.clamp(first_eos(mult_preds) + 1, max=max_pred).amax()
    e = first_eos(best_preds)
    ml = torch.minimum(torch.where(e < ps, e, ps).amax() + 1, ps)
    return torch.stack([ps, ml]).to(torch.int32)


class Engine:

    def __init__(self, state_dict: Dict[str, torch.Tensor], *, precision: str = "bf16", d_model: int = 256,
                 nhead: int = 8, n_layers: int = 6, d_ff: int = 2048, pad_id: int = 0, bos_id: int = 1,
                 eos_id: int = 2, device: Optional[torch.device] = None) -> None:
        if not torch.cuda.is_available():
            raise RuntimeError("conette_amd.Engine needs a ROCm GPU (no CPU fallback)")
        self.lib = load_library()
        self.device = torch.device("cuda", torch.cuda.current_device()) if device is None else torch.device(device)
        table = {"fp32": PREC_F32, "f32": PREC_F32, "bf16": PREC_BF16, "exact": PREC_F16X2, "f16x2": PREC_F16X2,
                 "f16": PREC_F16, "fp16": PREC_F16}
        head = precision.split(":", 1)[0]
        self.certified = head in ("certified", "certified-best")
        self.cert_order = head != "certified-best"
        base = precision
        if self.certified:
            base = precision.split(":", 1)[1] if ":" in precision else CERT_DEFAULT_BASE
            if base not in CERT_TOL:
                raise ValueError(f"certified: unknown base precision {base!r} (expected one of {tuple(CERT_TOL)})")
        self.base_precision = base
        if base == "mixed":
            self.precision, self.precision_dec = PREC_BF16, PREC_F16X2
        elif base == "mixed16":
            self.precision, self.precision_dec = PREC_F16, PREC_F16X2
        elif base == "bf16+f16dec":
            self.precision, self.precision_dec = PREC_BF16, PREC_F16
        else:
            if base not in table:
                raise ValueError(f"unknown precision {precision!r}" + (" (the experimental fp8 precision was withdrawn in round 6: "
                                 "profiles/r06_notes.md section 3)" if base == "fp8" else f" (expected one of {sorted(table)}, mixed, mixed16, "
                                 "bf16+f16dec, certified[:base])"))
            self.precision = self.precision_dec = table[base]
        self.precision_name = precision if (self.certified or base in ("mixed", "mixed16", "bf16+f16dec")) else {
            PREC_BF16: "bf16", PREC_F32: "fp32", PREC_F16X2: "exact", PREC_F16: "f16"}[self.precision]
        self.eos_id, self.pad_id = int(eos_id), int(pad_id)
        vocab = int(state_dict["model.decoder.classifier.weight"].shape[0])
        self.vocab_size = vocab
        self.d_model, self.nhead, self.n_layers, self.d_ff = d_model, nhead, n_layers, d_ff
        keep, names, ptrs, numel = [], [], [], []
        with torch.cuda.device(self.device):
            for k, v in state_dict.items():
                if not isinstance(v, torch.Tensor) or k == "_extra_state_":
                    continue
                if v.dtype == torch.bool:
                    v = v.to(torch.uint8)
                elif v.is_floating_point():
                    v = v.to(torch.float32)
                v = v.to(self.device).contiguous()
                keep.append(v)
                names.append(k.encode())
                ptrs.append(v.data_ptr())
                numel.append(v.numel())
            n = len(names)

            def create(prec: int) -> C.c_void_p:
                cfg = ConetteConfigC(prec, vocab, d_model, nhead, n_layers, d_ff, pad_id, bos_id, eos_id)
                handle = C.c_void_p()
                torch.cuda.synchronize(self.device)
                st = self.lib.conette_create(C.byref(cfg), n, (C.c_char_p * n)(*names), (C.c_void_p * n)(*ptrs),
                                             (C.c_int64 * n)(*numel), C.byref(handle))
                _check(st, "conette_create")
                torch.cuda.synchronize(self.device)
                return handle

            self._ctx = create(self.precision)
            self._ctx_dec = create(self.precision_dec) if self.precision_dec != self.precision else self._ctx
            self._ctx_x = None
            if self.certified:
                self._ctx_x = self._ctx_dec if self.precision_dec == PREC_F16X2 else create(PREC_F16X2)
        self.cert_stats = {"clips": 0, "recomputed": 0}
        self._ws: Dict[str, torch.Tensor] = {}
        self._dec_bufs: Dict[Any, Dict[str, Any]] = {}
        del keep

    def __del__(self) -> None:
        seen = []
        for c in (getattr(self, "_ctx", None), getattr(self, "_ctx_dec", None), getattr(self, "_ctx_x", None)):
            if c and all(c is not d for d in seen):
                seen.append(c)
                try:
                    self.lib.conette_destroy(c)
                except Exception:
                    pass
        self._ctx = self._ctx_dec = self._ctx_x = None

    def _workspace(self, key: str, nbytes: int) -> torch.Tensor:
        ws = self._ws.get(key)
        if ws is None or ws.numel() < nbytes:
            ws = torch.empty(int(nbytes), dtype=torch.uint8, device=self.device)
            self._ws[key] = ws
        return ws

    def frontend_logmel(self, wave: torch.Tensor) -> torch.Tensor:
        wave = wave.to(self.device, torch.float32).contiguous()
        b, l = wave.shape
        out = torch.empty((b, self.lib.conette_num_frames(l), N_MELS), dtype=torch.float32, device=self.device)
        _check(self.lib.conette_frontend_logmel(self._ctx, _ptr(wave), b, l, _ptr(out), _stream()), "frontend_logmel")
        return out

    def encode(self, wave: torch.Tensor, taps=False, out: Optional[Tuple[torch.Tensor, torch.Tensor]] = None,
               slot: int = 0, exact: bool = False):
        ctx = self._ctx
        if exact:
            if self._ctx_x is None:
                raise RuntimeError("encode(exact=True) needs a certified engine")
            ctx = self._ctx_x
        wave = wave.to(self.device, torch.float32).contiguous()
        b, l = wave.shape
        f, hs, ws_ = encoder_geometry(l)
        t = hs[3]
        if out is None:
            frame_embs = torch.empty((b, t, FEAT), dtype=torch.float32, device=self.device)
            clip = torch.empty((b, N_TAGS), dtype=torch.float32, device=self.device)
        else:
            frame_embs, clip = out
        need = self.lib.conette_encode_workspace_bytes(ctx, b, l)
        wsb = self._workspace(("xenc" if exact else "enc") + ("" if slot == 0 else str(slot)), need)
        tap_struct, tap_out = None, None
        if taps:
            dims = (96, 192, 384, 768)
            e = lambda *s: torch.empty(s, dtype=torch.float32, device=self.device)
            tap_out = {"logmel": e(b, f, N_MELS), "stem": e(b, hs[0], ws_[0], 96)}
            for i in range(4):
                tap_out[f"stage{i}_block0"] = e(b, hs[i], ws_[i], dims[i])
                tap_out[f"stage{i}"] = e(b, hs[i], ws_[i], dims[i])
                if i > 0:
                    tap_out[f"down{i}"] = e(b, hs[i], ws_[i], dims[i])
            tap_struct = EncodeTapsC()
            tap_struct.struct_bytes = C.sizeof(EncodeTapsC)
            tap_struct.logmel = tap_out["logmel"].data_ptr()
            tap_struct.stem = tap_out["stem"].data_ptr()
            for i in range(4):
                tap_struct.stage_block0[i] = tap_out[f"stage{i}_block0"].data_ptr()
                tap_struct.stage[i] = tap_out[f"stage{i}"].data_ptr()
                tap_struct.down[i] = tap_out[f"down{i}"].data_ptr() if i > 0 else 0
            if taps == "blocks":
                blk = 0
                for i, depth in enumerate((3, 3, 9, 3)):
                    for _ in range(depth):
                        tap_out[f"block{blk}"] = e(b, hs[i], ws_[i], dims[i])
                        tap_struct.block[blk] = tap_out[f"block{blk}"].data_ptr()
                        blk += 1
        st = self.lib.conette_encode(ctx, _ptr(wave), b, l, _ptr(frame_embs), _ptr(clip),
                                     C.byref(tap_struct) if tap_struct is not None else None, _ptr(wsb),
                                     wsb.numel(), _stream())
        _check(st, "conette_encode")
        if taps:
            return frame_embs, clip, tap_out
        return frame_embs, clip

    def _decode_buffers(self, b: int, t: int, beam: int, max_pred: int, s0: bool, trace: bool,
                        slot: int = 0, margins: bool = False, exact: bool = False) -> Dict[str, Any]:
        key = (b, t, beam, max_pred, s0, trace, slot, margins, exact)
        buf = self._dec_bufs.pop(key, None)
        if buf is not None:
            self._dec_bufs[key] = buf
        if buf is None:
            dev = self.device
            ldv = (self.vocab_size + 7) // 8 * 8
            e = lambda shape, dt: torch.empty(shape, dtype=dt, device=dev)
            buf = {
                "fe": e((b, t, FEAT), torch.float32), "lens": e((b,), torch.int32), "bos": e((b,), torch.int32),
                "forbid": e((self.vocab_size,), torch.uint8),
                "best_preds": e((b, max_pred), torch.int32), "best_lprobs": e((b,), torch.float32),
                "mult_preds": e((b, beam, max_pred), torch.int32), "mult_lprobs": e((b, beam), torch.float32),
                "sizes": e((2,), torch.int32),
                "step0": e((b * beam, ldv), torch.float32) if s0 else None,
                "trace_sel": e((max_pred, b, beam, 2), torch.int32) if trace else None,
                "trace_val": e((max_pred, b, beam), torch.float32) if trace else None,
                "margins": e((b, 2, max_pred + 1), torch.float32) if margins else None,
            }
            if len(self._dec_bufs) >= MAX_DECODE_GRAPHS:
                torch.cuda.synchronize(self.device)
                self._dec_bufs.pop(next(iter(self._dec_bufs)))
            self._dec_bufs[key] = buf
        return buf

    def decode(self, frame_embs: torch.Tensor, frame_lens: torch.Tensor, bos_ids: torch.Tensor,
               forbid_mask: Optional[torch.Tensor], beam: int, min_pred: int, max_pred: int,
               want_step0_logits: bool = False, want_trace: bool = False, clone: bool = True,
               slot: int = 0, want_margins: bool = False, exact: bool = False) -> Dict[str, torch.Tensor]:
        ctx = self._ctx_dec
        if exact:
            if self._ctx_x is None:
                raise RuntimeError("decode(exact=True) needs a certified engine")
            ctx = self._ctx_x
        b, t, _ = frame_embs.shape
        buf = self._decode_buffers(b, t, int(beam), int(max_pred), want_step0_logits, want_trace, slot, want_margins, exact)
        if frame_embs.data_ptr() != buf["fe"].data_ptr():
            buf["fe"].copy_(frame_embs, non_blocking=True)
        buf["lens"].copy_(frame_lens.to(torch.int32), non_blocking=True)
        buf["bos"].copy_(bos_ids.to(torch.int32), non_blocking=True)
        forbid_ptr = None
        if forbid_mask is not None:
            if forbid_mask.numel() != self.vocab_size:
                raise ValueError("forbid_mask must have vocab_size entries")
            buf["forbid"].copy_(forbid_mask.to(torch.uint8), non_blocking=True)
            forbid_ptr = buf["forbid"]
        need = self.lib.conette_decode_workspace_bytes(ctx, b, t, beam, max_pred)
        wsb = self._workspace(("xdec" if exact else "dec") + ("" if slot == 0 else str(slot)), need)
        st = self.lib.conette_decode(ctx, _ptr(buf["fe"]), _ptr(buf["lens"]), _ptr(buf["bos"]), _ptr(forbid_ptr),
                                     b, t, beam, min_pred, max_pred, _ptr(buf["best_preds"]), _ptr(buf["best_lprobs"]),
                                     _ptr(buf["mult_preds"]), _ptr(buf["mult_lprobs"]), _ptr(buf["sizes"]),
                                     _ptr(buf["step0"]), _ptr(buf["trace_sel"]), _ptr(buf["trace_val"]), _ptr(buf["margins"]),
                                     _ptr(wsb), wsb.numel(), _stream())
        _check(st, "conette_decode")
        cp = (lambda x: x.clone()) if clone else (lambda x: x)
        out = {k: cp(buf[k]) for k in ("best_preds", "best_lprobs", "mult_preds", "mult_lprobs", "sizes")}
        if want_step0_logits:
            out["step0_logits"] = cp(buf["step0"])[:, : self.vocab_size]
        if want_trace:
            out["trace_sel"] = cp(buf["trace_sel"])
            out["trace_val"] = cp(buf["trace_val"])
        if want_margins:
            out["margins"] = cp(buf["margins"])
        return out

    def uncertified(self, margins: torch.Tensor, best_lprobs: torch.Tensor, tol: Optional[Tuple[float, float, float]] = None,
                    beam: int = 2, order: Optional[bool] = None) -> torch.Tensor:
        tol = CERT_TOL[self.base_precision][cert_kind(beam)] if tol is None else tol
        return uncertified_mask(margins, best_lprobs, tol, self.cert_order if order is None else order)

    def caption_sizes(self, best_preds: torch.Tensor, mult_preds: torch.Tensor) -> torch.Tensor:
        return caption_sizes(best_preds, mult_preds, self.eos_id)

    def generate_certified(self, wave: Optional[torch.Tensor], frame_embs: torch.Tensor, frame_lens: torch.Tensor,
                           bos_ids: torch.Tensor, forbid_mask: Optional[torch.Tensor], beam: int, min_pred: int,
                           max_pred: int, tol: Optional[Tuple[float, float, float]] = None) -> Dict[str, torch.Tensor]:
        if not self.certified:
            raise RuntimeError("generate_certified needs Engine(precision='certified[:base]')")
        res = self.decode(frame_embs, frame_lens, bos_ids, forbid_mask, beam, min_pred, max_pred, want_margins=True)
        flag = self.uncertified(res["margins"], res["best_lprobs"], tol, beam)
        if wave is None and self.precision_dec == PREC_F16X2:
            flag = torch.zeros_like(flag)
        idx = torch.nonzero(flag).flatten()
        n = int(idx.numel())
        b = int(frame_embs.shape[0])
        self.cert_stats["clips"] += b
        self.cert_stats["recomputed"] += n
        res["recomputed"] = flag
        if n == 0:
            return res
        lens_d = frame_lens.to(self.device)
        bos_d = bos_ids.to(self.device)
        if wave is not None:
            fe_x, clip_x = self.encode(wave.index_select(0, idx), exact=True)
            res["recomputed_idx"], res["recomputed_clip_probs"] = idx, clip_x
        else:
            fe_x = frame_embs.to(self.device).index_select(0, idx)
        rx = self.decode(fe_x, lens_d.index_select(0, idx), bos_d.index_select(0, idx), forbid_mask, beam, min_pred, max_pred,
                         exact=True)
        for k in ("best_preds", "best_lprobs", "mult_preds", "mult_lprobs"):
            res[k].index_copy_(0, idx, rx[k])
        res["sizes"] = self.caption_sizes(res["best_preds"], res["mult_preds"])
        return res

    def encode_nonfinite(self) -> int:
        n = C.c_int32(0)
        _check(self.lib.conette_encode_nonfinite(self._ctx, _stream(), C.byref(n)), "conette_encode_nonfinite")
        return int(n.value)

    def forcing(self, frame_embs: torch.Tensor, frame_lens: torch.Tensor, caps_in: torch.Tensor) -> torch.Tensor:
        b, t, _ = frame_embs.shape
        cap_len = int(caps_in.shape[1])
        fe = frame_embs.to(self.device, torch.float32).contiguous()
        lens = frame_lens.to(self.device, torch.int32).contiguous()
        caps = caps_in.to(self.device, torch.int32).contiguous()
        out = torch.empty((b, cap_len, self.vocab_size), dtype=torch.float32, device=self.device)
        need = self.lib.conette_forcing_workspace_bytes(self._ctx_dec, b, t, cap_len)
        wsb = self._workspace("dec", need)
        st = self.lib.conette_forcing(self._ctx_dec, _ptr(fe), _ptr(lens), _ptr(caps), b, t, cap_len, _ptr(out), _ptr(wsb),
                                      wsb.numel(), _stream())
        _check(st, "conette_forcing")
        return out

    def score(self, frame_embs: torch.Tensor, frame_lens: torch.Tensor, caps_in: torch.Tensor, targets: torch.Tensor,
              caps_per_audio: int = 1, want_tokens: bool = True) -> Dict[str, Optional[torch.Tensor]]:
        from . import scoring
        n, t, _ = frame_embs.shape
        cpa, cap_len = int(caps_per_audio), int(caps_in.shape[1])
        if cpa < 1 or caps_in.ndim != 2 or tuple(caps_in.shape) != tuple(targets.shape) or caps_in.shape[0] != n * cpa:
            raise ValueError(f"score: caps_in {tuple(caps_in.shape)} / targets {tuple(targets.shape)} do not hold "
                             f"{n} x {cpa} captions of one length")
# ... 216 lines not shown
            need = self.lib.conette_decode_ensemble_workspace_bytes(ctx, b, t, beam, max_pred)
            wsb = self._workspace(f"ens{i}", need)
            recs[i] = ConetteMemberC(ctx, buf["fe"][i].data_ptr(), buf["bos"][i].data_ptr(), float(w64[i]), wsb.data_ptr(),
                                     wsb.numel())
        buf["lens"].copy_(frame_lens.to(torch.int32), non_blocking=True)
        forbid_ptr = None
        if forbid_mask is not None:
            if forbid_mask.numel() != self.vocab_size:
                raise ValueError("forbid_mask must have vocab_size entries")
            buf["forbid"].copy_(forbid_mask.to(torch.uint8), non_blocking=True)
            forbid_ptr = buf["forbid"]
        st = self.lib.conette_decode_ensemble(recs, m_n, rule, _ptr(buf["lens"]), _ptr(forbid_ptr), b, t, beam, int(min_pred), max_pred,
                                              _ptr(buf["best_preds"]), _ptr(buf["best_lprobs"]), _ptr(buf["mult_preds"]),
                                              _ptr(buf["mult_lprobs"]), _ptr(buf["sizes"]), _ptr(buf["trace_sel"]), _ptr(buf["trace_val"]),
                                              _ptr(buf["margins"]), _ptr(buf["step_logits"]), _stream())
        _check(st, "conette_decode_ensemble")
        cp = (lambda x: x.clone()) if clone else (lambda x: x)
        out = {k: cp(buf[k]) for k in ("best_preds", "best_lprobs", "mult_preds", "mult_lprobs", "sizes")}
        for k in ("trace_sel", "trace_val", "margins"):
            if buf[k] is not None:
                out[k] = cp(buf[k])
        if want_logits:
            out["step_logits"] = cp(buf["step_logits"])[..., : self.vocab_size]
        return out

    def decode_constrained(self, frame_embs: torch.Tensor, frame_lens: torch.Tensor, bos_ids: torch.Tensor,
                           forbid_mask: Optional[torch.Tensor], beam: int, min_pred: int, max_pred: int,
                           prefix: Optional[torch.Tensor] = None, prefix_lens: Optional[torch.Tensor] = None,
                           ban_mask: Optional[torch.Tensor] = None, no_repeat_ngram: int = 0, want_trace: bool = False,
                           want_logits: bool = False, exact: bool = False, check: bool = True) -> Dict[str, torch.Tensor]:
        return self._decode_steered("decode_constrained", frame_embs, frame_lens, bos_ids, forbid_mask, beam, min_pred, max_pred, prefix,
                                    prefix_lens, ban_mask, no_repeat_ngram, None, None, want_trace, want_logits, exact, check)

    def decode_required(self, frame_embs: torch.Tensor, frame_lens: torch.Tensor, bos_ids: torch.Tensor,
                        forbid_mask: Optional[torch.Tensor], beam: int, min_pred: int, max_pred: int,
                        prefix: Optional[torch.Tensor] = None, prefix_lens: Optional[torch.Tensor] = None,
                        ban_mask: Optional[torch.Tensor] = None, no_repeat_ngram: int = 0, req_tokens: Optional[torch.Tensor] = None,
                        req_groups: Optional[torch.Tensor] = None, want_trace: bool = False, want_logits: bool = False,
                        exact: bool = False, check: bool = True) -> Dict[str, torch.Tensor]:
        if (req_tokens is None) != (req_groups is None):
            raise ValueError("req_tokens and req_groups must be given together")
        if req_tokens is None:
            req_tokens = req_groups = torch.zeros((frame_embs.shape[0], 0), dtype=torch.int32)
        return self._decode_steered("decode_required", frame_embs, frame_lens, bos_ids, forbid_mask, beam, min_pred, max_pred, prefix,
                                    prefix_lens, ban_mask, no_repeat_ngram, req_tokens, req_groups, want_trace, want_logits, exact, check)

    def _decode_steered(self, entry, frame_embs, frame_lens, bos_ids, forbid_mask, beam, min_pred, max_pred, prefix, prefix_lens,
                        ban_mask, no_repeat_ngram, req_tokens, req_groups, want_trace, want_logits, exact, check):
        from . import constrained_search, required_search
        b, t, _ = frame_embs.shape
        max_pred = int(max_pred)
        pw = 0 if prefix is None else int(prefix.shape[1])
        if prefix is not None and (prefix.dim() != 2 or prefix.shape[0] != b):
            raise ValueError(f"prefix must be (batch, P), got {tuple(prefix.shape)}")
        rw = 0
        if req_tokens is not None:
            if req_tokens.dim() != 2 or req_tokens.shape[0] != b or tuple(req_groups.shape) != tuple(req_tokens.shape):
                raise ValueError(f"req_tokens and req_groups must both be (batch, width), got {tuple(req_tokens.shape)} and "
                                 f"{tuple(req_groups.shape)}")
            rw = int(req_tokens.shape[1])
            w, n = required_search.check_arguments(beam, no_repeat_ngram, max_pred, pw, rw)
        else:
            w, n = constrained_search.check_arguments(beam, no_repeat_ngram, max_pred, pw)
        ctx = self._ctx_dec
        if exact:
            if self._ctx_x is None:
                raise RuntimeError(f"{entry}(exact=True) needs a certified engine")
            ctx = self._ctx_x
        pre = plens = None
        if pw > 0:
            if prefix_lens is None:
                prefix_lens = torch.full((b,), pw, dtype=torch.int32)
            if prefix_lens.numel() != b:
                raise ValueError("prefix_lens must have one entry per clip")
            if check:
                ph, lh = prefix.cpu().long(), prefix_lens.cpu().long()
                if bool(((lh < 0) | (lh > pw)).any()):
                    raise ValueError(f"prefix_lens must lie in 0 .. {pw}")
                live = ph[torch.arange(pw)[None] < lh[:, None]]
                if bool(((live < 0) | (live >= self.vocab_size) | (live == self.eos_id) | (live == self.pad_id)).any()):
                    raise ValueError("prefix tokens must lie in the vocabulary and be neither <eos> nor pad")
            pre = prefix.to(self.device, torch.int32).contiguous()
            plens = prefix_lens.to(self.device, torch.int32).contiguous()
        fe = frame_embs.to(self.device, torch.float32).contiguous()
        lens_in = frame_lens.to(self.device, torch.int32).contiguous()
        bos = bos_ids.to(self.device, torch.int32).contiguous()
        masks = []
        for name, m in (("forbid_mask", forbid_mask), ("ban_mask", ban_mask)):
            if m is not None and m.numel() != self.vocab_size:
                raise ValueError(f"{name} must have vocab_size entries")
            masks.append(None if m is None else m.to(self.device, torch.uint8).contiguous())
        fm, bm = masks
        e = lambda shape, dt: torch.empty(shape, dtype=dt, device=self.device)
        o = {"best_preds": e((b, max_pred), torch.int32), "best_lprobs": e((b,), torch.float32),
             "mult_preds": e((b, w, max_pred), torch.int32), "mult_lprobs": e((b, w), torch.float32),
             "sizes": e((2,), torch.int32),
             "trace_sel": e((max_pred, b, w, 2), torch.int32) if want_trace else None,
             "trace_val": e((max_pred, b, w), torch.float32) if want_trace else None,
             "step_logits": e((max_pred, b * w, self.vocab_size), torch.float32) if want_logits else None}
        outs = (_ptr(o["best_preds"]), _ptr(o["best_lprobs"]), _ptr(o["mult_preds"]), _ptr(o["mult_lprobs"]), _ptr(o["sizes"]),
                _ptr(o["trace_sel"]), _ptr(o["trace_val"]), _ptr(o["step_logits"]))
        if req_tokens is None:
            need = self.lib.conette_decode_constrained_workspace_bytes(ctx, b, t, w, max_pred)
            wsb = self._workspace("xdec" if exact else "dec", need)
            st = self.lib.conette_decode_constrained(ctx, _ptr(fe), _ptr(lens_in), _ptr(bos), _ptr(fm), _ptr(pre), _ptr(plens), pw, _ptr(bm),
                                                     n, b, t, w, int(min_pred), max_pred, *outs, _ptr(wsb), wsb.numel(), _stream())
        else:
            rt = rg = None
            if rw > 0:
                if check:
                    self._check_req_tables(req_tokens, req_groups, bos_ids, prefix, prefix_lens, ban_mask, max_pred)
                rt = req_tokens.to(self.device, torch.int32).contiguous()
                rg = req_groups.to(self.device, torch.int32).contiguous()
            need = self.lib.conette_decode_required_workspace_bytes(ctx, b, t, w, max_pred)
            wsb = self._workspace("xdec" if exact else "dec", need)
            st = self.lib.conette_decode_required(ctx, _ptr(fe), _ptr(lens_in), _ptr(bos), _ptr(fm), _ptr(pre), _ptr(plens), pw, _ptr(bm),
                                                  n, _ptr(rt), _ptr(rg), rw, b, t, w, int(min_pred), max_pred, *outs, _ptr(wsb),
                                                  wsb.numel(), _stream())
        _check(st, "conette_" + entry)
        return {k: v for k, v in o.items() if v is not None}

    def _check_req_tables(self, req_tokens, req_groups, bos_ids, prefix, prefix_lens, ban_mask, max_pred) -> None:
        from . import required_search
        th, gh, bos = req_tokens.cpu().long(), req_groups.cpu().long(), bos_ids.cpu().long()
        if bool(((gh < -1) | (gh >= required_search.MAX_GROUPS)).any()):
            raise ValueError(f"req_groups must lie in -1 .. {required_search.MAX_GROUPS - 1}")
        ban = None if ban_mask is None else ban_mask.cpu().bool().numpy()
        for i in range(th.shape[0]):
            used = sorted(set(gh[i][gh[i] >= 0].tolist()))
            groups = [[int(x) for x in th[i][gh[i] == g].tolist()] for g in used]
            pre = []
            if prefix is not None:
                n_pre = int(prefix.shape[1]) if prefix_lens is None else int(prefix_lens.reshape(-1)[i])
                pre = [int(x) for x in prefix[i, :n_pre].cpu().tolist()]
            required_search.check_requirements(groups, int(bos[i]), vocab_size=self.vocab_size, max_pred=max_pred, eos_id=self.eos_id,
                                               pad_id=self.pad_id, ban=ban, prefix=pre)

    def decode_input_buffer(self, b: int, t: int, beam: int, max_pred: int, slot: int = 0, margins: bool = False,
                            exact: bool = False) -> torch.Tensor:
        return self._decode_buffers(b, t, int(beam), int(max_pred), False, False, slot, margins, exact)["fe"]

    def set_decode_graph(self, enabled: bool) -> None:
        _check(self.lib.conette_set_option(self._ctx_dec, OPT_DECODE_GRAPH, int(bool(enabled))), "set_option")

    def set_decode_fusion(self, enabled: bool) -> None:
        _check(self.lib.conette_set_option(self._ctx_dec, OPT_DECODE_FUSION, int(bool(enabled))), "set_option")

    def set_forcing_stepwise(self, enabled: bool) -> None:
        _check(self.lib.conette_set_option(self._ctx_dec, OPT_FORCING_STEPWISE, int(bool(enabled))), "set_option")

    def set_encode_reserved_cus(self, n: int) -> None:
        _check(self.lib.conette_set_option(self._ctx, OPT_ENCODE_RESERVED_CUS, int(n)), "set_option")

    def decode_graph_nodes(self) -> int:
        return int(self.lib.conette_decode_graph_nodes(self._ctx_dec))

    _DEC_CLASSES = ("dec_prepare", "dec_gemm", "dec_attn", "dec_misc", "search")

    def profile_enable(self, classes=()) -> None:
        mask_enc = mask_dec = 0
        for c in classes:
            bit = 1 << PROF_CLASSES.index(c)
            if c in self._DEC_CLASSES:
                mask_dec |= bit
            else:
                mask_enc |= bit
        if self._ctx_dec is self._ctx:
            _check(self.lib.conette_profile_enable(self._ctx, mask_enc | mask_dec), "profile_enable")
        else:
            _check(self.lib.conette_profile_enable(self._ctx, mask_enc), "profile_enable")
            _check(self.lib.conette_profile_enable(self._ctx_dec, mask_dec), "profile_enable")

    def profile_read(self) -> Dict[str, Any]:
        n = len(PROF_CLASSES)
        ms = (C.c_float * n)()
        cnt = (C.c_int32 * n)()
        _check(self.lib.conette_profile_read(self._ctx, ms, cnt), "profile_read")
        if self._ctx_dec is not self._ctx:
            _check(self.lib.conette_profile_read(self._ctx_dec, ms, cnt), "profile_read")
        return {PROF_CLASSES[i]: (float(ms[i]), int(cnt[i])) for i in range(n) if cnt[i] > 0}

    def resample(self, x: torch.Tensor, orig_sr: int, new_sr: int) -> torch.Tensor:
        if orig_sr == new_sr:
            return x
        shape = x.shape
        x2 = x.to(self.device, torch.float32).reshape(-1, shape[-1]).contiguous()
        n_out = self.lib.conette_resample_len(shape[-1], int(orig_sr), int(new_sr))
        out = torch.empty((x2.shape[0], n_out), dtype=torch.float32, device=self.device)
        _check(self.lib.conette_resample(_ptr(x2), x2.shape[0], shape[-1], int(orig_sr), int(new_sr), _ptr(out),
                                         _stream()), "conette_resample")
        return out.reshape(*shape[:-1], n_out)
```

include/conette_hip.h:

```cpp
#ifndef CONETTE_HIP_H
#define CONETTE_HIP_H

#include <stddef.h>
#include <stdint.h>

#ifdef __cplusplus
extern "C" {
#endif

#define CONETTE_ABI_VERSION 3

#define CONETTE_PREC_F32 0
#define CONETTE_PREC_BF16 1
#define CONETTE_PREC_F16X2 2


#define CONETTE_PREC_F16 4

typedef struct conette_ctx conette_ctx;

typedef struct conette_config {
  int32_t precision;
  int32_t vocab_size;
  int32_t d_model;
  int32_t nhead;
  int32_t n_layers;
  int32_t d_ff;
  int32_t pad_id;
  int32_t bos_id;
  int32_t eos_id;
  int32_t reserved[7];
} conette_config;

typedef struct conette_encode_taps {
  size_t struct_bytes;
  float* logmel;
  float* stem;
  float* stage_block0[4];
  float* stage[4];
  float* down[4];
  float* block[18];
} conette_encode_taps;

const char* conette_last_error(void);
int conette_abi_version(void);

int conette_create(const conette_config* cfg, int32_t n_tensors, const char* const* names,
                   const void* const* tensors, const int64_t* numel, conette_ctx** out);
void conette_destroy(conette_ctx* ctx);

int32_t conette_num_frames(int32_t n_samples);
int32_t conette_num_audio_frames(int32_t n_samples);

size_t conette_encode_workspace_bytes(const conette_ctx* ctx, int32_t batch, int32_t n_samples);
size_t conette_decode_workspace_bytes(const conette_ctx* ctx, int32_t batch, int32_t t_audio, int32_t beam,
                                      int32_t max_pred);

int conette_frontend_logmel(conette_ctx* ctx, const float* wave, int32_t batch, int32_t n_samples, float* out,
                            void* stream);

int conette_encode(conette_ctx* ctx, const float* wave, int32_t batch, int32_t n_samples, float* frame_embs,
                   float* clip_probs, const conette_encode_taps* taps, void* workspace, size_t workspace_bytes,
                   void* stream);

int conette_encode_nonfinite(conette_ctx* ctx, void* stream, int32_t* count);

int conette_decode(conette_ctx* ctx, const float* frame_embs, const int32_t* frame_lens, const int32_t* bos_ids,
                   const uint8_t* forbid_mask, int32_t batch, int32_t t_audio, int32_t beam,
                   int32_t min_pred, int32_t max_pred, int32_t* best_preds, float* best_lprobs,
                   int32_t* mult_preds, float* mult_lprobs, int32_t* out_sizes, float* step0_logits,
                   int32_t* trace_sel, float* trace_val, float* margins, void* workspace, size_t workspace_bytes,
                   void* stream);

size_t conette_forcing_workspace_bytes(const conette_ctx* ctx, int32_t batch, int32_t t_audio, int32_t cap_len);
int conette_forcing(conette_ctx* ctx, const float* frame_embs, const int32_t* frame_lens, const int32_t* caps_in,
                    int32_t batch, int32_t t_audio, int32_t cap_len, float* logits, void* workspace,
                    size_t workspace_bytes, void* stream);

size_t conette_score_workspace_bytes(const conette_ctx* ctx, int32_t n_audio, int32_t t_audio, int32_t caps_per_audio,
                                     int32_t cap_len);
int conette_score(conette_ctx* ctx, const float* frame_embs, const int32_t* frame_lens, const int32_t* caps_in,
                  const int32_t* targets, int32_t n_audio, int32_t t_audio, int32_t caps_per_audio, int32_t cap_len,
                  float* tok_lprobs, float* sum_lprobs, int32_t* n_tokens, void* workspace, size_t workspace_bytes,
                  void* stream);

size_t conette_align_workspace_bytes(const conette_ctx* ctx, int32_t n_audio, int32_t t_audio, int32_t caps_per_audio,
                                     int32_t cap_len, int32_t with_scores);
int conette_align(conette_ctx* ctx, const float* frame_embs, const int32_t* frame_lens, const int32_t* caps_in,
                  const int32_t* targets, int32_t n_audio, int32_t t_audio, int32_t caps_per_audio, int32_t cap_len,
                  uint32_t layer_mask, float* attn, float* attn_layers, float* tok_lprobs, float* sum_lprobs, int32_t* n_tokens,
                  void* workspace, size_t workspace_bytes, void* stream);

size_t conette_greedy_workspace_bytes(const conette_ctx* ctx, int32_t batch, int32_t t_audio, int32_t max_pred);
int conette_greedy(conette_ctx* ctx, const float* frame_embs, const int32_t* frame_lens, const int32_t* bos_ids,
                   const uint8_t* forbid_mask, int32_t batch, int32_t t_audio, int32_t min_pred, int32_t max_pred,
                   float* logits, int32_t* preds, int32_t* out_sizes, void* workspace, size_t workspace_bytes,
                   void* stream);

size_t conette_sample_workspace_bytes(const conette_ctx* ctx, int32_t batch, int32_t t_audio, int32_t n_samples,
                                      int32_t max_pred);
int conette_sample(conette_ctx* ctx, const float* frame_embs, const int32_t* frame_lens, const int32_t* bos_ids,
                   const uint8_t* forbid_mask, const float* uniforms, int32_t batch, int32_t t_audio, int32_t n_samples,
                   int32_t min_pred, int32_t max_pred, float temperature, int32_t top_k, float top_p, int32_t* preds,
                   float* sum_lprobs, int32_t* lens, int32_t* out_sizes, float* tok_lprobs, float* step_logits,
                   void* workspace, size_t workspace_bytes, void* stream);

size_t conette_decode_groups_workspace_bytes(const conette_ctx* ctx, int32_t batch, int32_t t_audio, int32_t n_groups,
                                             int32_t group_beam, int32_t max_pred);
int conette_decode_groups(conette_ctx* ctx, const float* frame_embs, const int32_t* frame_lens, const int32_t* bos_ids,
                          const uint8_t* forbid_mask, int32_t batch, int32_t t_audio, int32_t n_groups, int32_t group_beam,
                          float diversity_penalty, int32_t min_pred, int32_t max_pred, int32_t* best_preds, float* best_lprobs,
                          int32_t* mult_preds, float* mult_lprobs, int32_t* out_sizes, int32_t* trace_sel, float* trace_val,
                          float* step_logits, void* workspace, size_t workspace_bytes, void* stream);

#define CONETTE_COMBINE_LOGPROB 0
#define CONETTE_COMBINE_PROB 1
typedef struct conette_member {
  conette_ctx* ctx;
  const float* frame_embs;
  const int32_t* bos_ids;
  float weight;
  void* workspace;
  size_t workspace_bytes;
} conette_member;
size_t conette_decode_ensemble_workspace_bytes(const conette_ctx* ctx, int32_t batch, int32_t t_audio, int32_t beam,
                                               int32_t max_pred);
int conette_decode_ensemble(const conette_member* members, int32_t n_members, int32_t combine, const int32_t* frame_lens,
                            const uint8_t* forbid_mask, int32_t batch, int32_t t_audio, int32_t beam, int32_t min_pred,
                            int32_t max_pred, int32_t* best_preds, float* best_lprobs, int32_t* mult_preds, float* mult_lprobs,
                            int32_t* out_sizes, int32_t* trace_sel, float* trace_val, float* margins, float* step_logits,
                            void* stream);

size_t conette_decode_constrained_workspace_bytes(const conette_ctx* ctx, int32_t batch, int32_t t_audio, int32_t beam,
                                                  int32_t max_pred);
int conette_decode_constrained(conette_ctx* ctx, const float* frame_embs, const int32_t* frame_lens, const int32_t* bos_ids,
                               const uint8_t* forbid_mask, const int32_t* prefix, const int32_t* prefix_lens, int32_t prefix_width,
                               const uint8_t* ban_mask, int32_t no_repeat_ngram, int32_t batch, int32_t t_audio, int32_t beam,
                               int32_t min_pred, int32_t max_pred, int32_t* best_preds, float* best_lprobs, int32_t* mult_preds,
                               float* mult_lprobs, int32_t* out_sizes, int32_t* trace_sel, float* trace_val, float* step_logits,
                               void* workspace, size_t workspace_bytes, void* stream);

size_t conette_decode_required_workspace_bytes(const conette_ctx* ctx, int32_t batch, int32_t t_audio, int32_t beam, int32_t max_pred);
int conette_decode_required(conette_ctx* ctx, const float* frame_embs, const int32_t* frame_lens, const int32_t* bos_ids,
                            const uint8_t* forbid_mask, const int32_t* prefix, const int32_t* prefix_lens, int32_t prefix_width,
                            const uint8_t* ban_mask, int32_t no_repeat_ngram, const int32_t* req_tokens, const int32_t* req_groups,
                            int32_t req_width, int32_t batch, int32_t t_audio, int32_t beam, int32_t min_pred, int32_t max_pred,
                            int32_t* best_preds, float* best_lprobs, int32_t* mult_preds, float* mult_lprobs, int32_t* out_sizes,
                            int32_t* trace_sel, float* trace_val, float* step_logits, void* workspace, size_t workspace_bytes,
                            void* stream);

int conette_resample(const float* in, int32_t rows, int32_t n_in, int32_t orig_sr, int32_t new_sr, float* out,
                     void* stream);
int32_t conette_resample_len(int32_t n_in, int32_t orig_sr, int32_t new_sr);

int conette_stream_create_masked(const uint32_t* mask_words, int32_t n_words, void** out_stream);
int conette_stream_destroy(void* stream);

#define CONETTE_OPT_DECODE_GRAPH 1
#define CONETTE_OPT_DECODE_FUSION 2
#define CONETTE_OPT_ENCODE_RESERVED_CUS 3
#define CONETTE_OPT_FORCING_STEPWISE 4
#define CONETTE_OPT_SCORE_VSPLIT 5
int conette_set_option(conette_ctx* ctx, int32_t option, int32_t value);

int32_t conette_decode_graph_nodes(const conette_ctx* ctx);
#define CONETTE_MAX_DECODE_GRAPHS 64

#define CONETTE_PROF_FRONTEND 0
#define CONETTE_PROF_STEM 1
#define CONETTE_PROF_DWCONV_LN 2
#define CONETTE_PROF_PW1_GEMM 3
#define CONETTE_PROF_PW2_GEMM 4
#define CONETTE_PROF_DOWNSAMPLE 5
#define CONETTE_PROF_HEADS 6
#define CONETTE_PROF_DEC_PREPARE 7
#define CONETTE_PROF_DEC_GEMM 8
#define CONETTE_PROF_DEC_ATTN 9
#define CONETTE_PROF_DEC_MISC 10
#define CONETTE_PROF_SEARCH 11
#define CONETTE_PROF_NCLASS 12
int conette_profile_enable(conette_ctx* ctx, uint32_t class_mask);
int conette_profile_read(conette_ctx* ctx, float* ms, int32_t* counts);

#ifdef __cplusplus
}
#endif
#endif
```

Before: 13470 clips/s.

## Fuse log-mel frontend with the stem conv+LayerNorm into one kernel

Adds a fused kernel that computes log-mel frames into an LDS tile and immediately runs the MFMA stem convolution and LayerNorm on them, writing the stem activation directly. This removes the round trip of the full log-mel tensor through global memory and one kernel launch. The fused path is on by default unless a logmel tap is requested or the mel matrix does not fit in LDS, and a new option can turn it off. The trade-offs are a grid capped at the CU count and more LDS per block, which may reduce the frontend's parallelism.

```diff
diff --git a/conette-audio-captioning_amd/csrc/common.h b/conette-audio-captioning_amd/csrc/common.h
--- a/conette-audio-captioning_amd/csrc/common.h
+++ b/conette-audio-captioning_amd/csrc/common.h
@@ -71,6 +71,8 @@
 }
 
 typedef __attribute__((ext_vector_type(2))) float f32x2;
+
+__host__ __device__ constexpr int cn_rc2_chan(int m) { return (m & 19) | ((m & 4) << 1) | ((m & 8) >> 1); }
 typedef __attribute__((ext_vector_type(8))) _Float16 f16x8;
 typedef __attribute__((ext_vector_type(4))) unsigned u32x4;
 
diff --git a/conette-audio-captioning_amd/csrc/ctx.h b/conette-audio-captioning_amd/csrc/ctx.h
--- a/conette-audio-captioning_amd/csrc/ctx.h
+++ b/conette-audio-captioning_amd/csrc/ctx.h
@@ -98,6 +98,7 @@
   const float* cls_b;
   int n_cu;
   int enc_reserved_cus;
+  int enc_unfused;
   int forcing_stepwise;
   int score_vsplit;
   char* arena;
@@ -120,6 +121,9 @@
 };
 
 int cn_frontend(conette_ctx* ctx, const float* wave, int B, int L, float* out, hipStream_t s);
+bool cn_frontend_stem_fits(const conette_ctx* ctx);
+int cn_frontend_stem(conette_ctx* ctx, const float* wave, int B, int L, half_t* x, hipStream_t s);
+int cn_frontend_stem(conette_ctx* ctx, const float* wave, int B, int L, float* x, hipStream_t s);
 
 #define CN_BY_PRECISION(ctx, ...)                                                          \
   do {                                                                                     \
diff --git a/conette-audio-captioning_amd/csrc/decoder.hip b/conette-audio-captioning_amd/csrc/decoder.hip
--- a/conette-audio-captioning_amd/csrc/decoder.hip
+++ b/conette-audio-captioning_amd/csrc/decoder.hip
@@ -544,6 +544,10 @@
     ctx->enc_reserved_cus = value;
     return CN_OK;
   }
+  if (option == CONETTE_OPT_ENCODE_FUSION) {
+    ctx->enc_unfused = value ? 0 : 1;
+    return CN_OK;
+  }
   cn_set_error("set_option: unknown option %d", option);
   return CN_ERR_ARG;
 }
diff --git a/conette-audio-captioning_amd/csrc/encoder.hip b/conette-audio-captioning_amd/csrc/encoder.hip
--- a/conette-audio-captioning_amd/csrc/encoder.hip
+++ b/conette-audio-captioning_amd/csrc/encoder.hip
@@ -13,6 +13,7 @@
 #include "mlp_rs16.h"
 #include "mlp_sp.h"
 #include "down_fused.h"
+#include "stem_mfma.h"
 
 template <typename XT>
 __global__ __launch_bounds__(256) void cn_stem_mfma_kernel(const float* __restrict__ in, int F, int H0, long n_pos,
@@ -26,7 +27,7 @@
 #pragma unroll
   for (int t = 0; t < 3; ++t)
 #pragma unroll
-    for (int s = 0; s < 8; ++s) a[t][s] = w[(4 * (s >> 1) + 2 * h + (s & 1)) * 96 + 32 * t + cn_rc2_chan(j)];
+    for (int s = 0; s < 8; ++s) a[t][s] = cn_stem_a(w, t, s, j, h);
   __syncthreads();
   const long n_tiles = (n_pos + 31) >> 5;
   const long n_waves = (long)gridDim.x * 4;
@@ -44,59 +45,7 @@
       xv[i] = f32x2{0.f, 0.f};
       if (r >= 0 && r < F) xv[i] = *(const f32x2*)(in + ((size_t)b * F + r) * CN_N_MELS + 4 * wq + 2 * h);
     }
-    f32x16 acc[3];
-#pragma unroll
-    for (int t = 0; t < 3; ++t)
-#pragma unroll
-      for (int u = 0; u < 2; ++u) {
-        const f32x4 b0 = *(const f32x4*)(s_p + 32 * t + 16 * u + 8 * h), b1 = *(const f32x4*)(s_p + 32 * t + 16 * u + 8 * h + 4);
-#pragma unroll
-        for (int e = 0; e < 4; ++e) acc[t][8 * u + e] = b0[e], acc[t][8 * u + 4 + e] = b1[e];
-      }
-#pragma unroll
-    for (int s = 0; s < 8; ++s)
-#pragma unroll
-      for (int t = 0; t < 3; ++t) acc[t] = __builtin_amdgcn_mfma_f32_32x32x2f32(a[t][s], xv[s >> 1][s & 1], acc[t], 0, 0, 0);
-    float sum = 0.f;
-#pragma unroll
-    for (int t = 0; t < 3; ++t)
-#pragma unroll
-      for (int r = 0; r < 16; ++r) sum += acc[t][r];
-    sum += __shfl_xor(sum, 32);
-    const float mean = sum * (1.0f / 96.0f);
-    float v2 = 0.f;
-#pragma unroll
-    for (int t = 0; t < 3; ++t)
-#pragma unroll
-      for (int r = 0; r < 16; ++r) {
-        acc[t][r] -= mean;
-        v2 = fmaf(acc[t][r], acc[t][r], v2);
-      }
-    v2 += __shfl_xor(v2, 32);
-    const float rstd = 1.0f / sqrtf(v2 * (1.0f / 96.0f) + 1e-6f);
-    if (pos < n_pos) {
-      XT* o = out + (size_t)pos * 96 + 8 * h;
-#pragma unroll
-      for (int t = 0; t < 3; ++t)
-#pragma unroll
-        for (int u = 0; u < 2; ++u) {
-          const int ch = 32 * t + 16 * u + 8 * h;
-          float v[8];
-#pragma unroll
-          for (int q = 0; q < 2; ++q) {
-            const f32x4 lw = *(const f32x4*)(s_p + 96 + ch + 4 * q), lb = *(const f32x4*)(s_p + 192 + ch + 4 * q);
-#pragma unroll
-            for (int e = 0; e < 4; ++e) v[4 * q + e] = acc[t][8 * u + 4 * q + e] * rstd * lw[e] + lb[e];
-          }
-          if constexpr (sizeof(XT) == 2) {
-            *(cn_h8<XT>*)(o + 32 * t + 16 * u) = cn_h8<XT>{cn_from_f32<XT>(v[0]), cn_from_f32<XT>(v[1]), cn_from_f32<XT>(v[2]), cn_from_f32<XT>(v[3]),
-                                                          cn_from_f32<XT>(v[4]), cn_from_f32<XT>(v[5]), cn_from_f32<XT>(v[6]), cn_from_f32<XT>(v[7])};
-          } else {
-            *(f32x4*)(o + 32 * t + 16 * u) = f32x4{v[0], v[1], v[2], v[3]};
-            *(f32x4*)(o + 32 * t + 16 * u + 4) = f32x4{v[4], v[5], v[6], v[7]};
-          }
-        }
-    }
+    cn_stem_tile<XT>(a, xv, s_p, h, pos < n_pos ? out + (size_t)pos * 96 : (XT*)nullptr);
   }
 }
 
@@ -847,21 +796,23 @@
   T* y = (T*)ws.y;
   T* hbuf = (T*)ws.h;
   XT* const wsx = (XT*)ws.x;
+  const long n_pos = (long)B * g.H[0] * g.W[0];
+  const bool fe_fused = !ctx->enc_unfused && !(taps && taps->logmel) && cn_frontend_stem_fits(ctx);
   {
     CnProfScope ps(ctx, CONETTE_PROF_FRONTEND, s);
-    CN_TRY(cn_frontend(ctx, wave, B, L, ws.logmel, s));
-  }
-  if (taps) CN_TRY(tap_copy(taps->logmel, ws.logmel, (size_t)B * g.F * CN_N_MELS, s));
-  {
-    const long n_pos = (long)B * g.H[0] * g.W[0];
+    if (fe_fused) CN_TRY(cn_frontend_stem(ctx, wave, B, L, wsx, s));
+    else CN_TRY(cn_frontend(ctx, wave, B, L, ws.logmel, s));
+  }
+  if (!fe_fused) {
+    if (taps) CN_TRY(tap_copy(taps->logmel, ws.logmel, (size_t)B * g.F * CN_N_MELS, s));
     CnProfScope ps(ctx, CONETTE_PROF_STEM, s);
     const long n_tiles = (n_pos + 31) / 32;
     const unsigned grid = (unsigned)std::min<long>((n_tiles + 3) / 4, 8L * ctx->n_cu);
     hipLaunchKernelGGL((cn_stem_mfma_kernel<XT>), dim3(grid), dim3(256), 0, s, ws.logmel, g.F, g.H[0], n_pos, ctx->stem_w, ctx->stem_b,
                        ctx->stem_ln_w, ctx->stem_ln_b, wsx);
     CN_LAUNCH_CHECK();
-    if (taps) CN_TRY(tap_copy(taps->stem, wsx, (size_t)n_pos * 96, s));
-  }
+  }
+  if (taps) CN_TRY(tap_copy(taps->stem, wsx, (size_t)n_pos * 96, s));
   XT* xc = wsx;
   int blk = 0;
   for (int st = 0; st < 4; ++st) {
diff --git a/conette-audio-captioning_amd/csrc/frontend.hip b/conette-audio-captioning_amd/csrc/frontend.hip
--- a/conette-audio-captioning_amd/csrc/frontend.hip
+++ b/conette-audio-captioning_amd/csrc/frontend.hip
@@ -1,4 +1,6 @@
 #include "ctx.h"
+#include "stem_mfma.h"
+#include <algorithm>
 
 __device__ __forceinline__ float2 cmul(float2 a, float2 b) { return float2{a.x * b.x - a.y * b.y, a.x * b.y + a.y * b.x}; }
 __device__ __forceinline__ float2 cadd(float2 a, float2 b) { return float2{a.x + b.x, a.y + b.y}; }
@@ -41,6 +43,135 @@
 #define FE_MEL_LDS_MAX FE_FILL_BYTES
 static_assert(FE_STATIC_BYTES + FE_FILL_BYTES > FE_LDS_TOTAL - 768 && FE_STATIC_BYTES + FE_FILL_BYTES <= FE_LDS_TOTAL,
               "the log-mel block must own its compute unit's LDS");
+
+struct FeLane {
+  int m_lo[4], m_trip[4];
+  float m_sc[4], m_sh[4];
+  __device__ __forceinline__ int lo(int g) const { return m_lo[g]; }
+  __device__ __forceinline__ int trip(int g) const { return m_trip[g]; }
+  __device__ __forceinline__ float sc(int g) const { return m_sc[g]; }
+  __device__ __forceinline__ float sh(int g) const { return m_sh[g]; }
+};
+struct FeLaneLds {
+  const int* p;
+  __device__ __forceinline__ int lo(int g) const { return p[64 * g]; }
+  __device__ __forceinline__ int trip(int g) const { return p[64 * (4 + g)]; }
+  __device__ __forceinline__ float sc(int g) const { return __int_as_float(p[64 * (8 + g)]); }
+  __device__ __forceinline__ float sh(int g) const { return __int_as_float(p[64 * (12 + g)]); }
+};
+__device__ __forceinline__ FeLane fe_lane_setup(int lane, int mel_rows, const int* __restrict__ band, const float* __restrict__ bn_scale,
+                                                const float* __restrict__ bn_shift) {
+  FeLane fl;
+#pragma unroll
+  for (int g = 0; g < 4; ++g) {
+    const int m = lane + 64 * g;
+    const bool on = m < CN_N_MELS;
+    fl.m_sc[g] = on ? bn_scale[m] : 0.f;
+    fl.m_sh[g] = on ? bn_shift[m] : 0.f;
+    fl.m_lo[g] = on ? band[2 * m] : 0;
+    int nb = on ? band[2 * m + 1] - fl.m_lo[g] : 0;
+#pragma unroll
+    for (int d = 32; d > 0; d >>= 1) nb = max(nb, __shfl_xor(nb, d));
+    fl.m_trip[g] = min(nb, mel_rows);
+  }
+  return fl;
+}
+
+template <bool MEL_LDS, typename FL>
+__device__ __forceinline__ void fe_frame(const float* __restrict__ x, int L, int f, bool act, bool pair_loads, int lane,
+                                         const float* s_win, const float2* s_tw512, const float2* s_tw1024, float2* sx, float* sp,
+                                         const float* mc, const FL& fl, float (&res)[4]) {
+  float2 v[8];
+  if (act) {
+    const int p0 = f * CN_HOP - CN_N_FFT / 2;
+    if (pair_loads && p0 >= 0 && p0 + CN_N_FFT <= L) {
+#pragma unroll
+      for (int a = 0; a < 8; ++a) {
+        const int n2 = 2 * (64 * a + lane);
+        const float2 xv = *(const float2*)(x + p0 + n2);
+        const float2 wv2 = *(const float2*)(s_win + n2);
+        v[a] = float2{xv.x * wv2.x, xv.y * wv2.y};
+      }
+    } else {
+#pragma unroll
+      for (int a = 0; a < 8; ++a) {
+        const int n2 = 2 * (64 * a + lane);
+        int q0 = p0 + n2, q1 = q0 + 1;
+        q0 = q0 < 0 ? -q0 : (q0 >= L ? 2 * L - 2 - q0 : q0);
+        q1 = q1 < 0 ? -q1 : (q1 >= L ? 2 * L - 2 - q1 : q1);
+        v[a] = float2{x[q0] * s_win[n2], x[q1] * s_win[n2 + 1]};
+      }
+    }
+  } else {
+#pragma unroll
+    for (int a = 0; a < 8; ++a) v[a] = float2{0.f, 0.f};
+  }
+  dft8(v);
+#pragma unroll
+  for (int c = 1; c < 8; ++c) v[c] = cmul(v[c], s_tw512[lane * c]);
+#pragma unroll
+  for (int c = 0; c < 8; ++c) sx[c * FE_PITCH + lane] = v[c];
+  cn_wave_sync();
+  const int c = lane >> 3, lo3 = lane & 7;
+#pragma unroll
+  for (int a = 0; a < 8; ++a) v[a] = sx[c * FE_PITCH + 8 * a + lo3];
+  dft8(v);
+#pragma unroll
+  for (int cp = 1; cp < 8; ++cp) v[cp] = cmul(v[cp], s_tw512[8 * lo3 * cp]);
+  cn_wave_sync();
+#pragma unroll
+  for (int cp = 0; cp < 8; ++cp) sx[c * FE_PITCH + cp * 8 + lo3] = v[cp];
+  cn_wave_sync();
+#pragma unroll
+  for (int bp = 0; bp < 8; ++bp) v[bp] = sx[c * FE_PITCH + lo3 * 8 + bp];
+  dft8(v);
+  cn_wave_sync();
+#pragma unroll
+  for (int dp = 0; dp < 8; ++dp) sx[c + 8 * lo3 + 64 * dp] = v[dp];
+  cn_wave_sync();
+#pragma unroll
+  for (int j = 0; j < 8; ++j) {
+    const int k = lane + 64 * j;
+    const float2 A = sx[k];
+    const float2 Bz = sx[(512 - k) & 511];
+    const float2 E = float2{0.5f * (A.x + Bz.x), 0.5f * (A.y - Bz.y)};
+    const float2 O = float2{0.5f * (A.y + Bz.y), -0.5f * (A.x - Bz.x)};
+    const float2 X = cadd(E, cmul(s_tw1024[k], O));
+    sp[k] = X.x * X.x + X.y * X.y;
+  }
+  if (lane == 0) {
+    const float2 A = sx[0];
+    const float xr = A.x - A.y;
+    sp[512] = xr * xr;
+  }
+  cn_wave_sync();
+  if (act) {
+#pragma unroll
+    for (int g = 0; g < 4; ++g) {
+      const int m = lane + 64 * g;
+      if (m < CN_N_MELS) {
+        const int lo = fl.lo(g), trip = fl.trip(g);
+        float acc = 0.f;
+        int i = 0;
+        for (; i + 4 <= trip; i += 4) {
+          float p[4], w[4];
+#pragma unroll
+          for (int u = 0; u < 4; ++u) {
+            p[u] = sp[min(lo + i + u, CN_N_BINS - 1)];
+            w[u] = mc[(i + u) * CN_N_MELS + m];
+          }
+#pragma unroll
+          for (int u = 0; u < 4; ++u) acc = fmaf(p[u], w[u], acc);
+        }
+        for (; i < trip; ++i) acc = fmaf(sp[min(lo + i, CN_N_BINS - 1)], mc[i * CN_N_MELS + m], acc);
+        const float db = 10.0f * log10f(acc < 1e-10f ? 1e-10f : acc);
+        res[g] = db * fl.sc(g) + fl.sh(g);
+      }
+    }
+  }
+  cn_wave_sync();
+}
+
 template <bool MEL_LDS>
 __global__ __launch_bounds__(FE_NW * 64) void cn_logmel_kernel(const float* __restrict__ wave, int L, int F, int total, int mel_rows,
                                                         const float* __restrict__ window,
@@ -62,127 +193,111 @@
   for (int i = tid; i < 513; i += FE_NW * 64) s_tw1024[i] = tw1024[i];
   for (int i = tid; i < 1024; i += FE_NW * 64) s_win[i] = window[i];
   __syncthreads();
-  float2* sx = s_x[wv];
-  float* sp = s_p[wv];
-  int m_lo[4], m_trip[4];
-  float m_sc[4], m_sh[4];
-#pragma unroll
-  for (int g = 0; g < 4; ++g) {
-    const int m = lane + 64 * g;
-    const bool on = m < CN_N_MELS;
-    m_sc[g] = on ? bn_scale[m] : 0.f;
-    m_sh[g] = on ? bn_shift[m] : 0.f;
-    m_lo[g] = on ? band[2 * m] : 0;
-    int nb = on ? band[2 * m + 1] - m_lo[g] : 0;
-#pragma unroll
-    for (int d = 32; d > 0; d >>= 1) nb = max(nb, __shfl_xor(nb, d));
-    m_trip[g] = min(nb, mel_rows);
-  }
+  const FeLane fl = fe_lane_setup(lane, mel_rows, band, bn_scale, bn_shift);
   const bool pair_loads = (L & 1) == 0 && (((size_t)wave) & 7) == 0;
 
   for (int base = blockIdx.x * FE_NW; base < total; base += gridDim.x * FE_NW) {
     const int fr = base + wv;
     const bool act = fr < total;
-    float2 v[8];
-    if (act) {
-      const int b = fr / F, f = fr - b * F;
-      const float* x = wave + (size_t)b * L;
-      const int p0 = f * CN_HOP - CN_N_FFT / 2;
-      if (pair_loads && p0 >= 0 && p0 + CN_N_FFT <= L) {
-#pragma unroll
-        for (int a = 0; a < 8; ++a) {
-          const int n2 = 2 * (64 * a + lane);
-          const float2 xv = *(const float2*)(x + p0 + n2);
-          const float2 wv2 = *(const float2*)(s_win + n2);
-          v[a] = float2{xv.x * wv2.x, xv.y * wv2.y};
-        }
-      } else {
-#pragma unroll
-        for (int a = 0; a < 8; ++a) {
-          const int n2 = 2 * (64 * a + lane);
-          int q0 = p0 + n2, q1 = q0 + 1;
-          q0 = q0 < 0 ? -q0 : (q0 >= L ? 2 * L - 2 - q0 : q0);
-          q1 = q1 < 0 ? -q1 : (q1 >= L ? 2 * L - 2 - q1 : q1);
-          v[a] = float2{x[q0] * s_win[n2], x[q1] * s_win[n2 + 1]};
-        }
-      }
-    } else {
-#pragma unroll
-      for (int a = 0; a < 8; ++a) v[a] = float2{0.f, 0.f};
-    }
-    dft8(v);
-#pragma unroll
-    for (int c = 1; c < 8; ++c) v[c] = cmul(v[c], s_tw512[lane * c]);
-#pragma unroll
-    for (int c = 0; c < 8; ++c) sx[c * FE_PITCH + lane] = v[c];
-    cn_wave_sync();
-    const int c = lane >> 3, lo3 = lane & 7;
-#pragma unroll
-    for (int a = 0; a < 8; ++a) v[a] = sx[c * FE_PITCH + 8 * a + lo3];
-    dft8(v);
-#pragma unroll
-    for (int cp = 1; cp < 8; ++cp) v[cp] = cmul(v[cp], s_tw512[8 * lo3 * cp]);
-    cn_wave_sync();
-#pragma unroll
-    for (int cp = 0; cp < 8; ++cp) sx[c * FE_PITCH + cp * 8 + lo3] = v[cp];
-    cn_wave_sync();
-#pragma unroll
-    for (int bp = 0; bp < 8; ++bp) v[bp] = sx[c * FE_PITCH + lo3 * 8 + bp];
-    dft8(v);
-    cn_wave_sync();
-#pragma unroll
-    for (int dp = 0; dp < 8; ++dp) sx[c + 8 * lo3 + 64 * dp] = v[dp];
-    cn_wave_sync();
-#pragma unroll
-    for (int j = 0; j < 8; ++j) {
-      const int k = lane + 64 * j;
-      const float2 A = sx[k];
-      const float2 Bz = sx[(512 - k) & 511];
-      const float2 E = float2{0.5f * (A.x + Bz.x), 0.5f * (A.y - Bz.y)};
-      const float2 O = float2{0.5f * (A.y + Bz.y), -0.5f * (A.x - Bz.x)};
-      const float2 X = cadd(E, cmul(s_tw1024[k], O));
-      sp[k] = X.x * X.x + X.y * X.y;
-    }
-    if (lane == 0) {
-      const float2 A = sx[0];
-      const float xr = A.x - A.y;
-      sp[512] = xr * xr;
-    }
-    cn_wave_sync();
+    const int b = act ? fr / F : 0, f = fr - b * F;
+    float res[4];
+    fe_frame<MEL_LDS>(wave + (size_t)b * L, L, f, act, pair_loads, lane, s_win, s_tw512, s_tw1024, s_x[wv], s_p[wv],
+                      MEL_LDS ? s_mel : melC, fl, res);
     if (act) {
 #pragma unroll
       for (int g = 0; g < 4; ++g) {
         const int m = lane + 64 * g;
-        if (m < CN_N_MELS) {
-          const int lo = m_lo[g], trip = m_trip[g];
-          const float* mc = MEL_LDS ? s_mel : melC;
-          float acc = 0.f;
-          int i = 0;
-          for (; i + 4 <= trip; i += 4) {
-            float p[4], w[4];
-#pragma unroll
-            for (int u = 0; u < 4; ++u) {
-              p[u] = sp[min(lo + i + u, CN_N_BINS - 1)];
-              w[u] = mc[(i + u) * CN_N_MELS + m];
-            }
-#pragma unroll
-            for (int u = 0; u < 4; ++u) acc = fmaf(p[u], w[u], acc);
-          }
-          for (; i < trip; ++i) acc = fmaf(sp[min(lo + i, CN_N_BINS - 1)], mc[i * CN_N_MELS + m], acc);
-          const float db = 10.0f * log10f(acc < 1e-10f ? 1e-10f : acc);
-          out[(size_t)fr * CN_N_MELS + m] = db * m_sc[g] + m_sh[g];
-        }
+        if (m < CN_N_MELS) out[(size_t)fr * CN_N_MELS + m] = res[g];
       }
     }
-    cn_wave_sync();
-  }
-}
-
-int cn_frontend(conette_ctx* ctx, const float* wave, int B, int L, float* out, hipStream_t s) {
+  }
+}
+
+#define FE_TILE_FLOATS (FE_NW * CN_N_MELS)
+#define FE_STEM_TILES (FE_NW / 4 * 56 / 32)
+#define FE_STEM_STATIC_BYTES ((FE_TILE_FLOATS + 3 * 96 + 24 * 64 + 16 * 64) * 4)
+#define FE_STEM_FILL_BYTES (FE_FILL_BYTES - FE_STEM_STATIC_BYTES)
+static_assert(FE_NW == 16 && FE_STEM_TILES * 32 == FE_NW / 4 * 56, "a chunk's stem rows must be whole 32-position tiles");
+static_assert(FE_STEM_STATIC_BYTES % 16 == 0 && FE_STEM_FILL_BYTES > 0, "the stem's LDS is carved out of the fill");
+template <typename XT>
+__global__ __launch_bounds__(FE_NW * 64) void cn_logmel_stem_kernel(const float* __restrict__ wave, int L, int F, int H0, int n_chunks,
+                                                             int chunks_per_clip, int mel_rows, const float* __restrict__ window,
+                                                             const float2* __restrict__ tw512, const float2* __restrict__ tw1024,
+                                                             const float* __restrict__ melC, const int* __restrict__ band,
+                                                             const float* __restrict__ bn_scale, const float* __restrict__ bn_shift,
+                                                             const float* __restrict__ stem_w, const float* __restrict__ stem_b,
+                                                             const float* __restrict__ stem_ln_w, const float* __restrict__ stem_ln_b,
+                                                             XT* __restrict__ out) {
+  __shared__ float2 s_tw512[512];
+  __shared__ float2 s_tw1024[513];
+  __shared__ __attribute__((aligned(16))) float s_win[1024];
+  __shared__ float2 s_x[FE_NW][8 * FE_PITCH];
+  __shared__ float s_p[FE_NW][520];
+  __shared__ __attribute__((aligned(16))) float s_tile[FE_TILE_FLOATS];
+  __shared__ __attribute__((aligned(16))) float s_sp[3 * 96];
+  __shared__ float s_wa[24 * 64];
+  __shared__ int s_fl[16 * 64];
+  extern __shared__ __attribute__((aligned(16))) float s_mel[];
+  const int tid = threadIdx.x, lane = tid & 63;
+  const int wv = __builtin_amdgcn_readfirstlane(tid >> 6);
+  for (int i = tid; i < mel_rows * CN_N_MELS; i += FE_NW * 64) s_mel[i] = melC[i];
+  for (int i = tid; i < 512; i += FE_NW * 64) s_tw512[i] = tw512[i];
+  for (int i = tid; i < 513; i += FE_NW * 64) s_tw1024[i] = tw1024[i];
+  for (int i = tid; i < 1024; i += FE_NW * 64) s_win[i] = window[i];
+  for (int i = tid; i < 3 * 96; i += FE_NW * 64) s_sp[i] = i < 96 ? stem_b[i] : i < 192 ? stem_ln_w[i - 96] : stem_ln_b[i - 192];
+  for (int i = tid; i < 24 * 64; i += FE_NW * 64) s_wa[i] = cn_stem_a(stem_w, i >> 9, (i >> 6) & 7, i & 31, (i >> 5) & 1);
+  if (wv == 0) {
+    const FeLane r = fe_lane_setup(lane, mel_rows, band, bn_scale, bn_shift);
+#pragma unroll
+    for (int g = 0; g < 4; ++g) {
+      s_fl[64 * g + lane] = r.m_lo[g], s_fl[64 * (4 + g) + lane] = r.m_trip[g];
+      s_fl[64 * (8 + g) + lane] = __float_as_int(r.m_sc[g]), s_fl[64 * (12 + g) + lane] = __float_as_int(r.m_sh[g]);
+    }
+  }
+  __syncthreads();
+  const FeLaneLds fl{s_fl + lane};
+  const bool pair_loads = (L & 1) == 0 && (((size_t)wave) & 7) == 0;
+
+  for (int ck = blockIdx.x; ck < n_chunks; ck += gridDim.x) {
+    const int b = ck / chunks_per_clip, c = ck - b * chunks_per_clip;
+    const int f = FE_NW * c - 4 + wv;
+    const bool act = f >= 0 && f < F;
+    float res[4] = {0.f, 0.f, 0.f, 0.f};
+    if (act)
+      fe_frame<true>(wave + (size_t)b * L, L, f, true, pair_loads, lane, s_win, s_tw512, s_tw1024, s_x[wv], s_p[wv], s_mel, fl, res);
+    __syncthreads();
+#pragma unroll
+    for (int g = 0; g < 4; ++g) {
+      const int m = lane + 64 * g;
+      if (m < CN_N_MELS) s_tile[wv * CN_N_MELS + m] = res[g];
+    }
+    __syncthreads();
+    if (wv < FE_STEM_TILES && 4 * c + (32 * wv) / 56 < H0) {
+      const int h = lane >> 5, lp = 32 * wv + (lane & 31), rr = lp / 56, wq = lp - 56 * rr;
+      float a[3][8];
+#pragma unroll
+      for (int t = 0; t < 3; ++t)
+#pragma unroll
+        for (int s = 0; s < 8; ++s) a[t][s] = s_wa[(t * 8 + s) * 64 + lane];
+      f32x2 xv[4];
+#pragma unroll
+      for (int i = 0; i < 4; ++i) xv[i] = *(const f32x2*)(s_tile + (4 * rr + i) * CN_N_MELS + 4 * wq + 2 * h);
+      const int hh = 4 * c + rr;
+      cn_stem_tile<XT>(a, xv, s_sp, h, hh < H0 ? out + (((size_t)b * H0 + hh) * 56 + wq) * 96 : (XT*)nullptr);
+    }
+  }
+}
+
+static int fe_check(int L) {
   if (L <= CN_N_FFT / 2) {
     cn_set_error("frontend: n_samples=%d must exceed %d (reflect padding)", L, CN_N_FFT / 2);
     return CN_ERR_ARG;
   }
+  return CN_OK;
+}
+
+int cn_frontend(conette_ctx* ctx, const float* wave, int B, int L, float* out, hipStream_t s) {
+  CN_TRY(fe_check(L));
   const int F = L / CN_HOP + 1;
   const long total = (long)B * F;
   int grid = (int)((total + FE_NW - 1) / FE_NW);
@@ -201,3 +316,22 @@
   CN_LAUNCH_CHECK();
   return CN_OK;
 }
+
+bool cn_frontend_stem_fits(const conette_ctx* ctx) { return ctx->mel_rows * CN_N_MELS * 4 <= FE_STEM_FILL_BYTES; }
+
+template <typename XT>
+static int frontend_stem(conette_ctx* ctx, const float* wave, int B, int L, XT* x, hipStream_t s) {
+  CN_TRY(fe_check(L));
+  const int F = L / CN_HOP + 1, H0 = (F + 4) / 4 + 1;
+  const int chunks_per_clip = (H0 + FE_NW / 4 - 1) / (FE_NW / 4);
+  const long n_chunks = (long)B * chunks_per_clip;
+  const int grid = (int)std::min<long>(n_chunks, ctx->n_cu);
+  CN_TRY(cn_configure_lds((const void*)cn_logmel_stem_kernel<XT>, FE_STEM_FILL_BYTES));
+  hipLaunchKernelGGL(cn_logmel_stem_kernel<XT>, dim3(grid), dim3(FE_NW * 64), FE_STEM_FILL_BYTES, s, wave, L, F, H0, (int)n_chunks,
+                     chunks_per_clip, ctx->mel_rows, ctx->window, ctx->tw512, ctx->tw1024, ctx->melC, ctx->band, ctx->bn_scale,
+                     ctx->bn_shift, ctx->stem_w, ctx->stem_b, ctx->stem_ln_w, ctx->stem_ln_b, x);
+  CN_LAUNCH_CHECK();
+  return CN_OK;
+}
+int cn_frontend_stem(conette_ctx* ctx, const float* wave, int B, int L, half_t* x, hipStream_t s) { return frontend_stem(ctx, wave, B, L, x, s); }
+int cn_frontend_stem(conette_ctx* ctx, const float* wave, int B, int L, float* x, hipStream_t s) { return frontend_stem(ctx, wave, B, L, x, s); }
diff --git a/conette-audio-captioning_amd/csrc/mlp_rc2.h b/conette-audio-captioning_amd/csrc/mlp_rc2.h
--- a/conette-audio-captioning_amd/csrc/mlp_rc2.h
+++ b/conette-audio-captioning_amd/csrc/mlp_rc2.h
@@ -10,7 +10,6 @@
   static constexpr size_t STREAM_BYTES = (size_t)NSTEP * STEP_BYTES;
   static constexpr size_t TOTAL_BYTES = STREAM_BYTES + NT2 * 1024;
 };
-__host__ __device__ constexpr int cn_rc2_chan(int m) { return (m & 19) | ((m & 4) << 1) | ((m & 8) >> 1); }
 
 #define CN_MLP_XSCALE 0.5f
 template <typename HT> __device__ __forceinline__ float cn_gelu_mlp(float x) {
diff --git a/conette-audio-captioning_amd/csrc/stem_mfma.h b/conette-audio-captioning_amd/csrc/stem_mfma.h
--- /dev/null
+++ b/conette-audio-captioning_amd/csrc/stem_mfma.h
@@ -0,0 +1,63 @@
+#pragma once
+#include "common.h"
+
+__device__ __forceinline__ float cn_stem_a(const float* __restrict__ w , int t, int s, int j, int h) {
+  return w[(4 * (s >> 1) + 2 * h + (s & 1)) * 96 + 32 * t + cn_rc2_chan(j)];
+}
+
+template <typename XT>
+__device__ __forceinline__ void cn_stem_tile(const float (&a)[3][8], const f32x2 (&xv)[4], const float* s_p, int h, XT* o) {
+  f32x16 acc[3];
+#pragma unroll
+  for (int t = 0; t < 3; ++t)
+#pragma unroll
+    for (int u = 0; u < 2; ++u) {
+      const f32x4 b0 = *(const f32x4*)(s_p + 32 * t + 16 * u + 8 * h), b1 = *(const f32x4*)(s_p + 32 * t + 16 * u + 8 * h + 4);
+#pragma unroll
+      for (int e = 0; e < 4; ++e) acc[t][8 * u + e] = b0[e], acc[t][8 * u + 4 + e] = b1[e];
+    }
+#pragma unroll
+  for (int s = 0; s < 8; ++s)
+#pragma unroll
+    for (int t = 0; t < 3; ++t) acc[t] = __builtin_amdgcn_mfma_f32_32x32x2f32(a[t][s], xv[s >> 1][s & 1], acc[t], 0, 0, 0);
+  float sum = 0.f;
+#pragma unroll
+  for (int t = 0; t < 3; ++t)
+#pragma unroll
+    for (int r = 0; r < 16; ++r) sum += acc[t][r];
+  sum += __shfl_xor(sum, 32);
+  const float mean = sum * (1.0f / 96.0f);
+  float v2 = 0.f;
+#pragma unroll
+  for (int t = 0; t < 3; ++t)
+#pragma unroll
+    for (int r = 0; r < 16; ++r) {
+      acc[t][r] -= mean;
+      v2 = fmaf(acc[t][r], acc[t][r], v2);
+    }
+  v2 += __shfl_xor(v2, 32);
+  const float rstd = 1.0f / sqrtf(v2 * (1.0f / 96.0f) + 1e-6f);
+  if (o) {
+    o += 8 * h;
+#pragma unroll
+    for (int t = 0; t < 3; ++t)
+#pragma unroll
+      for (int u = 0; u < 2; ++u) {
+        const int ch = 32 * t + 16 * u + 8 * h;
+        float v[8];
+#pragma unroll
+        for (int q = 0; q < 2; ++q) {
+          const f32x4 lw = *(const f32x4*)(s_p + 96 + ch + 4 * q), lb = *(const f32x4*)(s_p + 192 + ch + 4 * q);
+#pragma unroll
+          for (int e = 0; e < 4; ++e) v[4 * q + e] = acc[t][8 * u + 4 * q + e] * rstd * lw[e] + lb[e];
+        }
+        if constexpr (sizeof(XT) == 2) {
+          *(cn_h8<XT>*)(o + 32 * t + 16 * u) = cn_h8<XT>{cn_from_f32<XT>(v[0]), cn_from_f32<XT>(v[1]), cn_from_f32<XT>(v[2]), cn_from_f32<XT>(v[3]),
+                                                        cn_from_f32<XT>(v[4]), cn_from_f32<XT>(v[5]), cn_from_f32<XT>(v[6]), cn_from_f32<XT>(v[7])};
+        } else {
+          *(f32x4*)(o + 32 * t + 16 * u) = f32x4{v[0], v[1], v[2], v[3]};
+          *(f32x4*)(o + 32 * t + 16 * u + 4) = f32x4{v[4], v[5], v[6], v[7]};
+        }
+      }
+  }
+}
diff --git a/conette-audio-captioning_amd/engine.py b/conette-audio-captioning_amd/engine.py
--- a/conette-audio-captioning_amd/engine.py
+++ b/conette-audio-captioning_amd/engine.py
@@ -48,6 +48,7 @@
 OPT_ENCODE_RESERVED_CUS = 3
 OPT_FORCING_STEPWISE = 4
 OPT_SCORE_VSPLIT = 5
+OPT_ENCODE_FUSION = 6
 MAX_DECODE_GRAPHS = 64
 PROF_CLASSES = ("frontend", "stem", "dwconv_ln", "pw1_gemm", "pw2_gemm", "downsample", "heads", "dec_prepare",
                 "dec_gemm", "dec_attn", "dec_misc", "search")
@@ -359,7 +360,7 @@
         return out
 
     def encode(self, wave: torch.Tensor, taps=False, out: Optional[Tuple[torch.Tensor, torch.Tensor]] = None,
-               slot: int = 0, exact: bool = False):
+               slot: int = 0, exact: bool = False, logmel_tap: bool = True):
         ctx = self._ctx
         if exact:
             if self._ctx_x is None:
@@ -388,7 +389,10 @@
                     tap_out[f"down{i}"] = e(b, hs[i], ws_[i], dims[i])
             tap_struct = EncodeTapsC()
             tap_struct.struct_bytes = C.sizeof(EncodeTapsC)
-            tap_struct.logmel = tap_out["logmel"].data_ptr()
+            if logmel_tap:
+                tap_struct.logmel = tap_out["logmel"].data_ptr()
+            else:
+                del tap_out["logmel"]
             tap_struct.stem = tap_out["stem"].data_ptr()
             for i in range(4):
                 tap_struct.stage_block0[i] = tap_out[f"stage{i}_block0"].data_ptr()
@@ -911,6 +915,11 @@
     def set_encode_reserved_cus(self, n: int) -> None:
         _check(self.lib.conette_set_option(self._ctx, OPT_ENCODE_RESERVED_CUS, int(n)), "set_option")
 
+    def set_encode_fusion(self, enabled: bool) -> None:
+        for ctx in (self._ctx, self._ctx_x):
+            if ctx is not None:
+                _check(self.lib.conette_set_option(ctx, OPT_ENCODE_FUSION, int(bool(enabled))), "set_option")
+
     def decode_graph_nodes(self) -> int:
         return int(self.lib.conette_decode_graph_nodes(self._ctx_dec))
 
@@ -918,6 +927,7 @@
 
     def profile_enable(self, classes=()) -> None:
         mask_enc = mask_dec = 0
+        self._prof_enabled = tuple(classes)
         for c in classes:
             bit = 1 << PROF_CLASSES.index(c)
             if c in self._DEC_CLASSES:
@@ -937,7 +947,8 @@
         _check(self.lib.conette_profile_read(self._ctx, ms, cnt), "profile_read")
         if self._ctx_dec is not self._ctx:
             _check(self.lib.conette_profile_read(self._ctx_dec, ms, cnt), "profile_read")
-        return {PROF_CLASSES[i]: (float(ms[i]), int(cnt[i])) for i in range(n) if cnt[i] > 0}
+        enabled = getattr(self, "_prof_enabled", ())
+        return {PROF_CLASSES[i]: (float(ms[i]), int(cnt[i])) for i in range(n) if cnt[i] > 0 or PROF_CLASSES[i] in enabled}
 
     def resample(self, x: torch.Tensor, orig_sr: int, new_sr: int) -> torch.Tensor:
         if orig_sr == new_sr:
diff --git a/include/conette_hip.h b/include/conette_hip.h
--- a/include/conette_hip.h
+++ b/include/conette_hip.h
@@ -161,6 +161,7 @@
 #define CONETTE_OPT_ENCODE_RESERVED_CUS 3
 #define CONETTE_OPT_FORCING_STEPWISE 4
 #define CONETTE_OPT_SCORE_VSPLIT 5
+#define CONETTE_OPT_ENCODE_FUSION 6
 int conette_set_option(conette_ctx* ctx, int32_t option, int32_t value);
 
 int32_t conette_decode_graph_nodes(const conette_ctx* ctx);
```

After: 13510 clips/s (median of 6 runs). About the same (+0.3%).
